# Zhiyu014/GNN-UDS

Hardware: AMD Instinct MI355X
Metric: graph-steps/sec (forward rollout), |V|=10k |E|=12k d=64 (higher is better)
Workload: dtype f32 storage/accumulate, GEMM operands as bf16 hi+lo split (3 MFMA products)

## Files before the change

### gnn_uds_amd/_lib.py

```python
import ctypes
import os

import numpy as np
import torch

_HERE = os.path.dirname(os.path.abspath(__file__))
LIB_PATH = os.environ.get('UDS_LIB_PATH') or os.path.join(_HERE, 'libuds_hip.so')

ABI_VERSION = 22
FLAG_EXACT_FP32, FLAG_REQUIRE_FUSED = 1, 2
PRECISION_FLAGS = {'bf16x3': 0, 'fp32': FLAG_EXACT_FP32}

ACT = {None: 0, 'linear': 0, 'relu': 1, 'tanh': 2, 'sigmoid': 3, 'hard_sigmoid': 4}
_KIND = {'GRU': 0, 'LSTM': 1}

_c_i64 = ctypes.c_int64
_c_int = ctypes.c_int
_c_ptr = ctypes.c_void_p

SYMBOLS = {
    'uds_abi_version': (_c_int, []),
    'uds_last_error': (ctypes.c_char_p, []),
    'uds_csr_create': (_c_int, [_c_ptr, _c_ptr, _c_i64, _c_i64, _c_i64, ctypes.POINTER(_c_ptr)]),
    'uds_csr_destroy': (_c_int, [_c_ptr]),
    'uds_csr_shape': (_c_int, [_c_ptr, ctypes.POINTER(_c_i64), ctypes.POINTER(_c_i64), ctypes.POINTER(_c_i64),
                               ctypes.POINTER(ctypes.c_int32)]),
    'uds_csr_row_order': (_c_int, [_c_ptr, _c_ptr]),
    'uds_dense_act': (_c_int, [_c_ptr, _c_i64, _c_ptr, _c_i64, _c_i64, _c_ptr, _c_ptr, _c_i64, _c_int, _c_ptr, _c_ptr,
                               _c_ptr, _c_ptr, _c_ptr, _c_ptr]),
    'uds_csr_spmm': (_c_int, [_c_ptr, _c_ptr, _c_ptr, _c_i64, _c_i64, _c_ptr, _c_int, _c_ptr, _c_ptr]),
    'uds_conv1d_causal': (_c_int, [_c_ptr, _c_i64, _c_i64, _c_i64, _c_i64, _c_ptr, _c_ptr, _c_i64, _c_i64, _c_i64, _c_int, _c_ptr,
                                   _c_ptr]),
    'uds_dense_cumsum_heads': (_c_int, [_c_ptr, _c_i64, _c_i64, _c_i64, _c_ptr, _c_ptr, _c_ptr, _c_int, _c_ptr, _c_ptr, _c_ptr]),
    'uds_recurrent_fused': (_c_int, [_c_ptr, _c_i64, _c_ptr, _c_ptr, _c_ptr, _c_i64, _c_i64, _c_i64, _c_int, _c_ptr, _c_ptr]),
    'uds_recurrent_fused_supported': (_c_int, [_c_i64, _c_int]),
    'uds_recurrent_forward': (_c_int, [_c_ptr, _c_ptr, _c_ptr, _c_i64, _c_i64, _c_i64, _c_i64, _c_int, _c_ptr, _c_ptr]),
    'uds_attn_sum_pool': (_c_int, [_c_ptr, _c_ptr, _c_i64, _c_i64, _c_i64, _c_ptr, _c_ptr]),
    'uds_attn_sum_pool_pair': (_c_int, [_c_ptr, _c_i64, _c_ptr, _c_i64, _c_ptr, _c_i64, _c_i64, _c_ptr, _c_ptr, _c_ptr]),
    'uds_attn_sum_pool_backward': (_c_int, [_c_ptr, _c_i64, _c_ptr, _c_i64, _c_ptr, _c_ptr, _c_ptr, _c_ptr, _c_i64, _c_i64, _c_ptr, _c_ptr, _c_ptr,
                                            _c_ptr, _c_ptr]),
    'uds_dropout': (_c_int, [_c_ptr, _c_i64, ctypes.c_float, ctypes.c_uint64, ctypes.c_uint64, _c_ptr, _c_ptr]),
    'uds_recurrent_forward_train': (_c_int, [_c_ptr, _c_ptr, _c_ptr, _c_i64, _c_i64, _c_i64, _c_i64, _c_int, _c_ptr, _c_ptr, _c_ptr]),
    'uds_recurrent_backward': (_c_int, [_c_ptr, _c_ptr, _c_ptr, _c_ptr, _c_ptr, _c_ptr, _c_i64, _c_i64, _c_i64, _c_int, _c_ptr, _c_ptr, _c_ptr]),
    'uds_recurrent_bwd_packed_bytes': (_c_i64, [_c_i64, _c_int]),
    'uds_recurrent_pack_bwd': (_c_int, [_c_ptr, _c_i64, _c_int, _c_ptr, _c_ptr]),
    'uds_recurrent_backward_h': (_c_int, [_c_ptr, _c_ptr, _c_ptr, _c_ptr, _c_ptr, _c_ptr, _c_i64, _c_i64, _c_i64, _c_i64, _c_int, _c_ptr, _c_ptr,
                                          _c_ptr]),
    'uds_rowgemm_packed_bytes': (_c_i64, [_c_i64, _c_i64]),
    'uds_rowgemm_pack': (_c_int, [_c_ptr, _c_i64, _c_i64, _c_ptr, _c_ptr]),
    'uds_gat_aggregate_masked': (_c_int, [_c_ptr, _c_ptr, _c_ptr, _c_ptr, _c_ptr, _c_ptr, _c_i64, _c_i64, _c_int, _c_ptr, _c_ptr]),
    'uds_gat_aggregate_coef': (_c_int, [_c_ptr, _c_ptr, _c_ptr, _c_ptr, _c_ptr, _c_ptr, _c_i64, _c_i64, _c_int, _c_ptr, _c_ptr]),
    'uds_diffusion_forward': (_c_int, [_c_ptr, _c_ptr, _c_ptr, _c_ptr, _c_ptr, _c_i64, _c_i64, _c_int, _c_ptr, _c_ptr]),
    'uds_diffusion_backward_workspace_floats': (_c_i64, [_c_i64, _c_i64, _c_i64, _c_i64]),
    'uds_diffusion_backward': (_c_int, [_c_ptr, _c_ptr, _c_ptr, _c_ptr, _c_ptr, _c_ptr, _c_ptr, _c_ptr, _c_ptr, _c_ptr, _c_i64, _c_i64,
                                        _c_i64, _c_int, _c_ptr, _c_ptr, _c_ptr, _c_ptr]),
    'uds_diffusion_forward_m': (_c_int, [_c_ptr, _c_ptr, _c_ptr, _c_ptr, _c_ptr, _c_i64, _c_i64, _c_i64, _c_int, _c_ptr, _c_ptr]),
    'uds_diffusion_backward_m_workspace_floats': (_c_i64, [_c_i64, _c_i64, _c_i64, _c_i64]),
    'uds_diffusion_backward_m': (_c_int, [_c_ptr, _c_ptr, _c_ptr, _c_ptr, _c_ptr, _c_ptr, _c_ptr, _c_ptr, _c_ptr, _c_i64, _c_i64, _c_i64,
                                          _c_int, _c_ptr, _c_ptr, _c_ptr, _c_ptr]),
    'uds_halo_pack': (_c_int, [_c_ptr, _c_i64, _c_ptr, _c_i64, _c_i64, _c_i64, _c_ptr, _c_i64, _c_ptr, _c_i64, _c_ptr, _c_ptr]),
    'uds_halo_unpack': (_c_int, [_c_ptr, _c_i64, _c_i64, _c_ptr, _c_i64, _c_ptr, _c_i64, _c_ptr, _c_i64, _c_ptr, _c_i64, _c_ptr]),
    'uds_halo_pack_all': (_c_int, [_c_ptr, _c_i64, _c_ptr, _c_i64, _c_i64, _c_i64, _c_ptr, _c_i64, _c_ptr, _c_i64, _c_ptr, _c_ptr, _c_i64,
                                   _c_ptr, _c_ptr]),
    'uds_halo_unpack_all': (_c_int, [_c_ptr, _c_i64, _c_i64, _c_ptr, _c_i64, _c_ptr, _c_i64, _c_ptr, _c_ptr, _c_i64, _c_ptr, _c_i64, _c_ptr,
                                     _c_i64, _c_ptr]),
    'uds_halo_pack_clear_all': (_c_int, [_c_ptr, _c_i64, _c_ptr, _c_i64, _c_i64, _c_i64, _c_ptr, _c_i64, _c_ptr, _c_i64, _c_ptr, _c_ptr,
                                         _c_i64, _c_ptr, _c_ptr]),
    'uds_halo_accumulate_all': (_c_int, [_c_ptr, _c_i64, _c_i64, _c_ptr, _c_ptr, _c_i64, _c_ptr, _c_i64, _c_ptr, _c_i64, _c_ptr, _c_ptr,
                                         _c_i64, _c_ptr, _c_i64, _c_ptr, _c_i64, _c_ptr]),
    'uds_remainder_packed_bytes': (_c_i64, [_c_i64, _c_i64]),
    'uds_remainder_pack': (_c_int, [_c_ptr, _c_i64, _c_i64, _c_ptr, _c_ptr]),
    'uds_remainder_workspace_bytes': (_c_i64, [_c_i64, _c_i64, _c_i64, _c_i64]),
    'uds_remainder_forward_dense': (_c_int, [_c_ptr, _c_i64, _c_i64, _c_ptr, _c_i64, _c_ptr, _c_ptr, _c_int, _c_i64, _c_i64, _c_ptr, _c_ptr, _c_ptr]),
    'uds_remainder_forward': (_c_int, [_c_ptr, _c_i64, _c_i64, _c_ptr, _c_i64, _c_i64, _c_ptr, _c_ptr, _c_ptr]),
    'uds_rowgemm_forward': (_c_int, [_c_ptr, _c_i64, _c_i64, _c_i64, _c_i64, _c_ptr, _c_ptr, _c_i64, _c_i64, _c_i64, _c_int, _c_ptr, _c_ptr]),
    'uds_rowgemm_forward_pair': (_c_int, [_c_ptr, _c_i64, _c_ptr, _c_ptr, _c_ptr, _c_ptr, _c_i64, _c_ptr, _c_ptr, _c_ptr, _c_i64, _c_i64, _c_i64, _c_i64,
                                          _c_i64, _c_i64, _c_int, _c_ptr]),
    'uds_rowgemm_forward_cat': (_c_int, [_c_ptr, _c_i64, _c_ptr, _c_i64, _c_i64, _c_i64, _c_i64, _c_ptr, _c_ptr, _c_i64, _c_i64, _c_i64, _c_int,
                                         _c_ptr, _c_i64, _c_i64, _c_ptr]),
    'uds_dense_cumsum': (_c_int, [_c_ptr, _c_i64, _c_i64, _c_i64, _c_ptr, _c_ptr, _c_ptr, _c_int, _c_ptr, _c_ptr]),
    'uds_conv_stack_plan': (_c_int, [_c_i64, _c_i64, _c_i64, _c_int, _c_ptr, _c_ptr, _c_ptr]),
    'uds_conv_stack_forward': (_c_int, [_c_ptr, _c_i64, _c_i64, _c_i64, _c_ptr, _c_i64, _c_ptr, _c_ptr]),
    'uds_cumsum_act': (_c_int, [_c_ptr, _c_ptr, _c_i64, _c_i64, _c_i64, _c_i64, _c_int, _c_ptr, _c_ptr]),
    'uds_flow_balance': (_c_int, [_c_ptr, _c_ptr, _c_ptr, _c_i64, _c_ptr, _c_ptr, _c_ptr, _c_ptr, _c_ptr]),
    'uds_gat_workspace_floats': (_c_i64, [_c_i64, _c_i64, _c_i64]),
    'uds_gat_forward': (_c_int, [_c_ptr, _c_ptr, _c_i64, _c_ptr, _c_i64, _c_i64, _c_ptr, _c_ptr, _c_ptr, _c_ptr, _c_i64,
                                 _c_int, _c_ptr, _c_ptr, _c_ptr]),
    'uds_gat_aggregate': (_c_int, [_c_ptr, _c_ptr, _c_ptr, _c_ptr, _c_ptr, _c_i64, _c_i64, _c_int, _c_ptr, _c_ptr]),
    'uds_gat_backward': (_c_int, [_c_ptr, _c_ptr, _c_ptr, _c_ptr, _c_ptr, _c_ptr, _c_ptr, _c_ptr, _c_ptr, _c_i64, _c_i64, _c_ptr,
                                  _c_ptr, _c_ptr, _c_ptr, _c_ptr, _c_ptr]),
    'uds_gat_backward_coef': (_c_int, [_c_ptr, _c_ptr, _c_ptr, _c_ptr, _c_ptr, _c_ptr, _c_ptr, _c_ptr, _c_ptr, _c_ptr, _c_i64, _c_i64, _c_ptr,
                                       _c_ptr, _c_ptr, _c_ptr, _c_ptr, _c_ptr]),
    'uds_gat_aggregate_ex': (_c_int, [_c_ptr, _c_ptr, _c_ptr, _c_ptr, _c_ptr, _c_ptr, _c_ptr, _c_i64, _c_i64, _c_int, _c_ptr, _c_ptr]),
    'uds_gat_backward_ex': (_c_int, [_c_ptr, _c_ptr, _c_ptr, _c_ptr, _c_ptr, _c_ptr, _c_ptr, _c_ptr, _c_ptr, _c_ptr, _c_ptr, _c_i64, _c_i64,
                                     _c_ptr, _c_ptr, _c_ptr, _c_ptr, _c_ptr, _c_ptr]),
    'uds_gat_aggregate_heads': (_c_int, [_c_ptr, _c_ptr, _c_ptr, _c_ptr, _c_ptr, _c_ptr, _c_ptr, _c_i64, _c_i64, _c_i64, _c_int, _c_int, _c_ptr,
                                         _c_ptr, _c_ptr]),
    'uds_gat_backward_heads': (_c_int, [_c_ptr, _c_ptr, _c_ptr, _c_ptr, _c_ptr, _c_ptr, _c_ptr, _c_ptr, _c_ptr, _c_ptr, _c_ptr, _c_i64, _c_i64,
                                        _c_i64, _c_int, _c_ptr, _c_ptr, _c_ptr, _c_ptr, _c_ptr, _c_ptr]),
    'uds_csr_sddmm': (_c_int, [_c_ptr, _c_ptr, _c_ptr, _c_i64, _c_i64, _c_ptr, _c_ptr]),
    'uds_wgrad_workspace_floats': (_c_i64, [_c_i64, _c_i64, _c_i64, _c_int]),
    'uds_wgrad': (_c_int, [_c_ptr, _c_ptr, _c_i64, _c_i64, _c_i64, _c_i64, _c_i64, _c_i64, _c_int, _c_ptr, _c_ptr, _c_ptr, _c_ptr]),
    'uds_network_create': (_c_int, [_c_ptr, _c_ptr, _c_ptr, _c_ptr, ctypes.POINTER(_c_ptr)]),
    'uds_network_destroy': (_c_int, [_c_ptr]),
    'uds_network_prepare': (_c_int, [_c_ptr, _c_i64, _c_i64]),
    'uds_network_plan_info': (_c_int, [_c_ptr, _c_ptr]),
    'uds_tile_plan_create': (_c_int, [_c_ptr] * 8 + [_c_i64, _c_i64] + [ctypes.c_int32] * 4 + [ctypes.POINTER(_c_ptr)]),
    'uds_tile_plan_destroy': (_c_int, [_c_ptr]),
    'uds_tile_plan_sizes': (_c_int, [_c_ptr, ctypes.POINTER(_c_i64), ctypes.POINTER(_c_i64), _c_ptr]),
    'uds_tile_plan_copy': (_c_int, [_c_ptr, _c_ptr, _c_ptr]),
    'uds_tile_plan_blocks': (_c_int, [_c_ptr, _c_ptr, ctypes.POINTER(_c_i64)]),
    'uds_roll_update': (_c_int, [_c_ptr] * 7 + [_c_i64, _c_ptr, _c_i64, _c_ptr, _c_i64, _c_i64, _c_i64, _c_int, _c_ptr, _c_ptr, _c_ptr, _c_ptr]),
    'uds_predict_tail': (_c_int, [_c_ptr] * 9 + [_c_i64, _c_i64, _c_ptr, _c_ptr, _c_ptr]),
    'uds_predict_tail_workspace_floats': (_c_i64, [_c_i64, _c_i64, _c_i64, _c_i64]),
    'uds_predict_tail_backward': (_c_int, [_c_ptr] * 9 + [_c_i64, _c_i64] + [_c_ptr] * 8),
    'uds_fit_tail': (_c_int, [_c_ptr] * 15 + [_c_i64, _c_i64, _c_i64, _c_int] + [_c_ptr] * 5),
    'uds_fit_tail_workspace_floats': (_c_i64, [_c_i64, _c_i64, _c_i64, _c_i64]),
    'uds_fit_tail_backward': (_c_int, [_c_ptr] * 15 + [_c_i64, _c_i64, _c_i64, _c_int] + [_c_ptr] * 7),
    'uds_spatial_workspace_floats': (_c_i64, [_c_ptr, _c_i64, _c_i64, _c_i64]),
    'uds_spatial_packed_bytes': (_c_i64, []),
    'uds_spatial_pack_weights': (_c_int, [_c_ptr, _c_i64, _c_i64, _c_i64, _c_i64, _c_ptr, _c_ptr]),
    'uds_spatial_layer_forward': (_c_int, [_c_ptr, _c_ptr, _c_ptr, _c_i64, _c_ptr, _c_i64, _c_i64, _c_i64, _c_i64, _c_int,
                                           _c_int, _c_ptr, _c_ptr, _c_ptr, _c_ptr]),
    'uds_spatial_layer_forward_rem': (_c_int, [_c_ptr, _c_ptr, _c_ptr, _c_i64, _c_ptr, _c_i64, _c_ptr, _c_ptr, _c_i64, _c_i64, _c_i64, _c_int, _c_int,
                                      _c_ptr, _c_ptr, _c_ptr, _c_ptr]),
    'uds_spatial_layer_forward_split': (_c_int, [_c_ptr, _c_ptr, _c_ptr, _c_i64, _c_ptr, _c_i64, _c_ptr, _c_i64, _c_ptr, _c_i64, _c_i64,
                                                 _c_i64, _c_i64, _c_int, _c_int, _c_ptr, _c_ptr, _c_ptr, _c_ptr]),
}


class SpatialParams(ctypes.Structure):
    _fields_ = [(n, _c_ptr) for n in ('xe_k', 'xe_b', 'ex_k', 'ex_b', 'ne_n_val', 'ne_e_val',
                                      'gx_k', 'gx_as', 'gx_an', 'gx_b', 'ge_k', 'ge_as', 'ge_an', 'ge_b', 'packed')]


class UdsError(RuntimeError):
    pass


_lib = None


def load():
    global _lib
    if _lib is not None:
        return _lib
    if not os.path.exists(LIB_PATH):
        raise ImportError('%s is missing: the HIP engine is not built (run `python -m gnn_uds_amd.build`); '
                          'gnn_uds_amd has no CPU fallback' % LIB_PATH)
    lib = ctypes.CDLL(LIB_PATH)
    for name, (res, args) in SYMBOLS.items():
        fn = getattr(lib, name)
        fn.restype = res
        fn.argtypes = args
    if lib.uds_abi_version() != ABI_VERSION:
        raise ImportError('libuds_hip.so ABI %d, binding expects %d' % (lib.uds_abi_version(), ABI_VERSION))
    _lib = lib
    return lib


def _check(rc, what):
    if rc != 0:
        msg = load().uds_last_error()
        raise UdsError('%s failed (%d): %s' % (what, rc, msg.decode() if msg else '?'))


def _dev(t, name, allow_none=False):
    if t is None:
        if allow_none:
            return None
        raise UdsError('%s is required' % name)
    if not isinstance(t, torch.Tensor):
        raise UdsError('%s must be a torch.Tensor, got %r' % (name, type(t)))
    if not t.is_cuda:
        raise UdsError('%s is on %s: gnn_uds_amd runs on the MI355X only and has no CPU fallback' % (name, t.device))
    if t.dtype != torch.float32:
        raise UdsError('%s must be float32, got %s' % (name, t.dtype))
    if not t.is_contiguous():
        raise UdsError('%s must be contiguous' % name)
    _same_device(t.device.index, name)
    return t.data_ptr()


def _current_device():
    if not torch.cuda.is_available():
        raise UdsError('no HIP device is visible: gnn_uds_amd runs on the MI355X only and has no CPU fallback')
    return torch.cuda.current_device()


def _same_device(index, what):
    cur = _current_device()
    if index is not None and index != cur:
        raise UdsError('%s lives on cuda:%d but the current device is cuda:%d: call torch.cuda.set_device(%d) (one process per GPU) '
                       'or wrap the call in `with torch.cuda.device(%d):`' % (what, index, cur, index, index))


def _dev_i32(t, name):
    if not isinstance(t, torch.Tensor) or not t.is_cuda or t.dtype != torch.int32 or not t.is_contiguous():
        raise UdsError('%s must be a contiguous int32 HIP tensor' % name)
    _same_device(t.device.index, name)
    return t.data_ptr()


def _stream():
    return torch.cuda.current_stream().cuda_stream


def _nothing_to_launch(t, name, result):
    _dev(t, name)
    return result


def _out(out, shape, like, name):
    if out is None:
        return torch.empty(shape, device=like.device, dtype=torch.float32)
    if tuple(out.shape) != tuple(shape) or out.device != like.device:
        raise UdsError('%s must be %r on %s, got %r on %s' % (name, tuple(shape), like.device, tuple(out.shape), out.device))
    _dev(out, name)
    return out


class CsrHandle:

    def __init__(self, csr):
        lib = load()
        self.n_rows, self.n_cols, self.nnz = int(csr.n_rows), int(csr.n_cols), int(csr.nnz)
        rowptr = np.ascontiguousarray(csr.rowptr, dtype=np.int32)
        col = np.ascontiguousarray(csr.col, dtype=np.int32)
        h = _c_ptr()
        self.device = _current_device()
        _check(lib.uds_csr_create(rowptr.ctypes.data, col.ctypes.data, self.n_rows, self.n_cols, self.nnz,
                                  ctypes.byref(h)), 'uds_csr_create')
        self._h = h
        self._rowptr, self._col = rowptr, col
        self._t = None

    def transposed(self, device):
        if self._t is None:
            rows = np.repeat(np.arange(self.n_rows, dtype=np.int64), np.diff(self._rowptr.astype(np.int64)))
            cols = self._col.astype(np.int64)
            order = np.lexsort((rows, cols))
            t_rowptr = np.zeros(self.n_cols + 1, dtype=np.int64)
            np.add.at(t_rowptr, cols + 1, 1)
            t_rowptr = np.cumsum(t_rowptr)

            class _T:
                pass
            t = _T()
            t.n_rows, t.n_cols, t.nnz = self.n_cols, self.n_rows, self.nnz
            t.rowptr, t.col = t_rowptr.astype(np.int32), rows[order].astype(np.int32)
            self._t = (CsrHandle(t), order.astype(np.int32))
        h, perm = self._t
        if not isinstance(perm, torch.Tensor) or perm.device != torch.device(device):
            perm = torch.as_tensor(np.asarray(perm.cpu() if isinstance(perm, torch.Tensor) else perm), dtype=torch.int32,
                                   device=device)
            self._t = (h, perm)
        return h, perm

    @property
    def ptr(self):
        _same_device(self.device, 'this CSR handle')
        return self._h

    def row_order(self):
        out = np.empty(self.n_rows, dtype=np.int32)
        _check(load().uds_csr_row_order(self._h, out.ctypes.data), 'uds_csr_row_order')
        return out

    def max_degree(self):
        md = ctypes.c_int32()
        _check(load().uds_csr_shape(self._h, None, None, None, ctypes.byref(md)), 'uds_csr_shape')
        return md.value

    def __del__(self):
        h, self._h = getattr(self, '_h', None), None
        if h is not None and _lib is not None:
            _lib.uds_csr_destroy(h)


class NetworkHandle:

    def __init__(self, graph):
        lib = load()
        self.graph = graph
        self.adj = CsrHandle(graph.adj)
        self.edge_adj = CsrHandle(graph.edge_adj)
        self.inc_n = CsrHandle(graph.inc_n)
        self.inc_e = CsrHandle(graph.inc_e)
        h = _c_ptr()
        self.device = _current_device()
        _check(lib.uds_network_create(self.adj.ptr, self.edge_adj.ptr, self.inc_n.ptr, self.inc_e.ptr, ctypes.byref(h)),
               'uds_network_create')
        self._h = h
        self._prepared = {(64, 64)}

    @property
    def ptr(self):
        _same_device(self.device, 'this network handle')
        return self._h

    def prepare(self, fx, fe):
        key = (int(fx), int(fe))
        if key not in self._prepared:
            _check(load().uds_network_prepare(self.ptr, key[0], key[1]), 'uds_network_prepare')
            self._prepared.add(key)

    def plan_info(self):
        info = np.zeros(8, dtype=np.int32)
        _check(load().uds_network_plan_info(self._h, info.ctypes.data), 'uds_network_plan_info')
        keys = ('fused', 'node_tiles', 'link_tiles', 'p_cap', 'q_cap', 'meta_cap', 'lds_bytes', 't_code')
        out = dict(zip(keys, (int(v) for v in info)))
        out['t_node'], out['t_link'] = out['t_code'] // 1000, out['t_code'] % 1000
        return out

    def __del__(self):
        h, self._h = getattr(self, '_h', None), None
        if h is not None and _lib is not None:
            _lib.uds_network_destroy(h)


def tile_plan(graph, t_node=48, t_link=48, p_limit=0, q_limit=0, blocks=False):
    lib = load()
    arrs = []
    for c in (graph.adj, graph.edge_adj, graph.inc_n, graph.inc_e):
        arrs += [np.ascontiguousarray(c.rowptr, dtype=np.int32), np.ascontiguousarray(c.col, dtype=np.int32)]
    h = _c_ptr()
    _check(lib.uds_tile_plan_create(*[a.ctypes.data for a in arrs], graph.n_node, graph.n_edge, t_node, t_link,
                                    p_limit, q_limit, ctypes.byref(h)), 'uds_tile_plan_create')
    try:
        nt, pl = _c_i64(), _c_i64()
        caps = np.zeros(3, dtype=np.int32)
        _check(lib.uds_tile_plan_sizes(h, ctypes.byref(nt), ctypes.byref(pl), caps.ctypes.data), 'uds_tile_plan_sizes')
        hdr = np.zeros((nt.value, 8), dtype=np.int32)
        pool = np.zeros(pl.value, dtype=np.int32)
        _check(lib.uds_tile_plan_copy(h, hdr.ctypes.data, pool.ctypes.data), 'uds_tile_plan_copy')
        blk = None
        if blocks:
            stride = _c_i64()
            if lib.uds_tile_plan_blocks(h, None, ctypes.byref(stride)) == 0:
                blk = np.zeros((nt.value, stride.value), dtype=np.int32)
                _check(lib.uds_tile_plan_blocks(h, blk.ctypes.data, ctypes.byref(stride)), 'uds_tile_plan_blocks')
    finally:
        lib.uds_tile_plan_destroy(h)
    out = dict(p_cap=int(caps[0]), q_cap=int(caps[1]), meta_cap=int(caps[2]))
    if blocks:
        out['blocks'] = blk
    return hdr, pool, out


def dense_act(xa, kernel, bias=None, act='linear', xb=None, attn=None):
    lib = load()
    fa = xa.shape[-1]
    fb = 0 if xb is None else xb.shape[-1]
    rows = xa.numel() // fa
    fo = kernel.shape[-1]
    if kernel.shape[0] != fa + fb:
        raise UdsError('kernel has %d input features, inputs give %d' % (kernel.shape[0], fa + fb))
    if xb is not None and xb.shape[:-1] != xa.shape[:-1]:
        raise UdsError('xa %r and xb %r disagree on leading dims' % (tuple(xa.shape), tuple(xb.shape)))
    out = torch.empty(xa.shape[:-1] + (fo,), device=xa.device, dtype=torch.float32)
    s_self = s_nbr = None
    if attn is not None:
        s_self = torch.empty(xa.shape[:-1], device=xa.device, dtype=torch.float32)
        s_nbr = torch.empty_like(s_self)
    if rows == 0:
        return _nothing_to_launch(xa, 'xa', (out, s_self, s_nbr) if attn is not None else out)
    _check(lib.uds_dense_act(_dev(xa, 'xa'), fa, _dev(xb, 'xb', True), fb, rows, _dev(kernel, 'kernel'),
                             _dev(bias, 'bias', True), fo, ACT[act],
                             _dev(attn[0], 'a_self') if attn else None, _dev(attn[1], 'a_nbr') if attn else None,
                             _dev(out, 'out'), _dev(s_self, 's_self', True), _dev(s_nbr, 's_nbr', True), _stream()),
           'uds_dense_act')
    return (out, s_self, s_nbr) if attn is not None else out


def conv1d_causal(x, kernel, bias=None, dilation=1, act='linear'):
    lib = load()
    if x.dim() != 4 or kernel.dim() != 3 or kernel.shape[1] != x.shape[-1]:
        raise UdsError('conv1d_causal: x %r / kernel %r' % (tuple(x.shape), tuple(kernel.shape)))
    B, T, R, F = x.shape
    taps, _, H = kernel.shape
    out = torch.empty((B, T, R, H), device=x.device, dtype=torch.float32)
    if out.numel() == 0:
        return _nothing_to_launch(x, 'x', out)
    _check(lib.uds_conv1d_causal(_dev(x, 'x'), B, T, R, F, _dev(kernel, 'kernel'), _dev(bias, 'bias', True), taps, dilation, H,
                                 ACT[act], _dev(out, 'out'), _stream()), 'uds_conv1d_causal')
    return out


def recurrent_fused_supported(F, kind):
    return bool(load().uds_recurrent_fused_supported(int(F), _KIND[kind]))


def recurrent_pack(kernel, recurrent_kernel):
    G = recurrent_kernel.shape[1] // 64
    if tuple(recurrent_kernel.shape) != (64, G * 64) or G not in (3, 4) or (kernel is not None and kernel.shape[1] != G * 64):
        raise UdsError('recurrent_pack: kernel %r / recurrent kernel %r (F x G*64 and 64 x G*64 with G = 3 or 4)'
                       % (None if kernel is None else tuple(kernel.shape), tuple(recurrent_kernel.shape)))
    mats = [recurrent_kernel] if kernel is None else [kernel, recurrent_kernel]
    return torch.cat([rowgemm_pack(m[:, 64 * g:64 * (g + 1)].contiguous()) for m in mats for g in range(G)]).contiguous()


def recurrent_fused(x, packed, b_in, b_rec, kind, projected=False):
    lib = load()
    B, T, R, F = x.shape
    out = torch.empty((B, T, R, 64), device=x.device, dtype=torch.float32)
    if out.numel():
        _check(lib.uds_recurrent_fused(_dev(x, 'x'), 0 if projected else F, packed.data_ptr(), _dev(b_in, 'b_in', True), _dev(b_rec, 'b_rec', True),
                                       B, T, R, _KIND[kind], _dev(out, 'out'), _stream()), 'uds_recurrent_fused')
    return out


def attn_sum_pool(x, attn_kernel):
    lib = load()
    B, R, F = x.shape
    k = attn_kernel.reshape(-1).contiguous()
    if k.numel() != F:
        raise UdsError('attn_sum_pool: x %r, attn_kernel %r' % (tuple(x.shape), tuple(attn_kernel.shape)))
    out = torch.empty((B, F), device=x.device, dtype=torch.float32)
    if B:
        _check(lib.uds_attn_sum_pool(_dev(x, 'x'), _dev(k, 'attn_kernel'), B, R, F, _dev(out, 'out'), _stream()), 'uds_attn_sum_pool')
    return out


def _pool_pair_shapes(what, x, e, attn_kernel):
    if x.dim() != 3 or (e is not None and (e.dim() != 3 or e.shape[0] != x.shape[0] or e.shape[2] != x.shape[2])) or attn_kernel.numel() != x.shape[2]:
        raise UdsError('%s: x %r, e %r, attn_kernel %r' % (what, tuple(x.shape), None if e is None else tuple(e.shape), tuple(attn_kernel.shape)))
    if e is not None and e.shape[1] == 0:
        e = None
    return x.shape[0], x.shape[1], 0 if e is None else e.shape[1], x.shape[2], e, attn_kernel.reshape(-1).contiguous()


def attn_sum_pool_pair(x, e, attn_kernel, want_stat=False):
    lib = load()
    B, Rx, Re, F, e, k = _pool_pair_shapes('attn_sum_pool_pair', x, e, attn_kernel)
    out = torch.empty((B, F), device=x.device, dtype=torch.float32)
    stat = torch.empty((B, 2), device=x.device, dtype=torch.float32) if want_stat else None
    if B:
        _check(lib.uds_attn_sum_pool_pair(_dev(x, 'x'), Rx, _dev(e, 'e', True), Re, _dev(k, 'attn_kernel'), B, F, _dev(out, 'out'),
                                          _dev(stat, 'stat', True), _stream()), 'uds_attn_sum_pool_pair')
    return (out, stat) if want_stat else out


def attn_sum_pool_backward(x, e, attn_kernel, out, stat, grad, want_dx=True, want_de=True, want_dk=True, dx=None, de=None, dk=None, dk_ws=None):
    lib = load()
    B, Rx, Re, F, e, k = _pool_pair_shapes('attn_sum_pool_backward', x, e, attn_kernel)
    if tuple(out.shape) != (B, F) or tuple(stat.shape) != (B, 2) or tuple(grad.shape) != (B, F):
        raise UdsError('attn_sum_pool_backward: out %r, stat %r, grad %r for B=%d, F=%d' % (tuple(out.shape), tuple(stat.shape), tuple(grad.shape), B, F))
    dx = _out(dx, (B, Rx, F), x, 'dx') if want_dx else None
    de = _out(de, (B, Re, F), x, 'de') if want_de and e is not None else None
    dk = _out(dk, (F,), x, 'dk') if want_dk else None
    dk_ws = _out(dk_ws, (B, F), x, 'dk_ws') if want_dk else None
    if dx is not None or de is not None or dk is not None:
        _check(lib.uds_attn_sum_pool_backward(_dev(x, 'x'), Rx, _dev(e, 'e', True), Re, _dev(k, 'attn_kernel'), _dev(out, 'out'), _dev(stat, 'stat'),
                                              _dev(grad, 'grad'), B, F, _dev(dx, 'dx', True), _dev(de, 'de', True), _dev(dk_ws, 'dk_ws', True),
                                              _dev(dk, 'dk', True), _stream()), 'uds_attn_sum_pool_backward')
    return dx, de, dk


def dropout(x, rate, seed, offset):
    lib = load()
    x = x.contiguous()
    out = torch.empty_like(x)
    if out.numel():
        _check(lib.uds_dropout(_dev(x, 'x'), x.numel(), float(rate), int(seed) & 0xFFFFFFFFFFFFFFFF, int(offset) & 0xFFFFFFFFFFFFFFFF,
                               _dev(out, 'out'), _stream()), 'uds_dropout')
    return out


def _recurrent_forward(xp, recurrent_kernel, recurrent_bias, kind, train):
    lib = load()
    B, T, R, GH = xp.shape
    G = {'GRU': 3, 'LSTM': 4}[kind]
    H = GH // G
    if GH != G * H or tuple(recurrent_kernel.shape) != (H, GH):
        raise UdsError('recurrent_forward: xp %r, recurrent kernel %r for a %s' % (tuple(xp.shape), tuple(recurrent_kernel.shape), kind))
    out = torch.empty((B, T, R, H), device=xp.device, dtype=torch.float32)
    c = torch.empty_like(out) if train and kind == 'LSTM' else None
    if out.numel():
        entry = 'uds_recurrent_forward_train' if train else 'uds_recurrent_forward'
        _check(getattr(lib, entry)(_dev(xp, 'xp'), _dev(recurrent_kernel, 'recurrent_kernel'), _dev(recurrent_bias, 'recurrent_bias', True),
                                   B, T, R, H, _KIND[kind], _dev(out, 'out'), *([_dev(c, 'c', True)] if train else []), _stream()), entry)
    return out, c


def recurrent_forward_train(xp, recurrent_kernel, recurrent_bias, kind):
    return _recurrent_forward(xp, recurrent_kernel, recurrent_bias, kind, True)


RECURRENT_TRAIN_WIDTHS = tuple(range(16, 129, 16))


def recurrent_bwd_route(units):
    if units == 64:
        return 'uds_recurrent_backward'
    return 'uds_recurrent_backward_h' if units in RECURRENT_TRAIN_WIDTHS else None


# ... 852 lines not shown
```

### gnn_uds_amd/csrc/kernels_fused.hpp

```cpp
#pragma once
#include <hip/hip_runtime.h>
#include <stdint.h>

#include <type_traits>

#include "kernels_dense.hpp"
#include "kernels_sparse.hpp"
#include "tile_plan.hpp"

namespace uds {

typedef __attribute__((ext_vector_type(8))) __bf16 bf16x8;
typedef __attribute__((ext_vector_type(4))) float f32x4;

constexpr int FUSED_H = 32;
constexpr int FUSED_D = 64;
constexpr int FUSED_WAVES = 8;
constexpr int FUSED_U = 4;
constexpr int SEC_STRIDE = FUSED_H + 4;

struct FusedSide {
  const float *prim_in, *sec_in;
  const float *prim_in2, *sec_in2;
  float *out;
  const uint4 *w_small, *w_big;
  const uint4 *w_big32, *w_small32;
  const float *b_small, *a_self, *a_nbr, *b_out, *ne_val;
  int n_prim_glob, n_sec_glob;
  const float *rem;
};

struct FusedArgs {
  FusedSide side[2];
  const int32_t *hdr, *pool;
  const int32_t *blocks;
  int n_tiles, S, chunk, p_cap, q_cap, meta_cap, act, side_mask;
  unsigned long long *dbg;
};

__device__ __forceinline__ int frag_k(int t, int qd, int jj) { return 32 * t + (jj < 4 ? 4 * qd + jj : 16 + 4 * qd + (jj - 4)); }

__global__ void k_pack_weight_frags(const float *__restrict__ W, int K, int F_out, uint4 *__restrict__ out) {
  const int MB = F_out / 16, KT = K / 32;
  const int idx = blockIdx.x * blockDim.x + threadIdx.x;
  if (idx >= KT * MB * 64) return;
  const int lane = idx & 63, m = (idx >> 6) % MB, t = (idx >> 6) / MB;
  const int qd = lane >> 4, f = 16 * m + (lane & 15);
  bf16x8 hi, lo;
#pragma unroll
  for (int jj = 0; jj < 8; ++jj) {
    const float w = W[(int64_t)frag_k(t, qd, jj) * F_out + f];
    const __bf16 h = (__bf16)w;
    hi[jj] = h;
    lo[jj] = (__bf16)(w - (float)h);
  }
  out[((t * MB + m) * 2 + 0) * 64 + lane] = __builtin_bit_cast(uint4, hi);
  out[((t * MB + m) * 2 + 1) * 64 + lane] = __builtin_bit_cast(uint4, lo);
}

__global__ void k_pack_weight_frags32(const float *__restrict__ W, int K, int F_out, uint4 *__restrict__ out) {
  const int MB = F_out / 32, KT = K / 16;
  const int idx = blockIdx.x * blockDim.x + threadIdx.x;
  if (idx >= KT * MB * 64) return;
  const int lane = idx & 63, m = (idx >> 6) % MB, t = (idx >> 6) / MB;
  const int hf = lane >> 5, f = 32 * m + (lane & 31);
  bf16x8 hi, lo;
#pragma unroll
  for (int jj = 0; jj < 8; ++jj) {
    const float w = W[(int64_t)(16 * t + 8 * hf + jj) * F_out + f];
    const __bf16 h = (__bf16)w;
    hi[jj] = h;
    lo[jj] = (__bf16)(w - (float)h);
  }
  out[((t * MB + m) * 2 + 0) * 64 + lane] = __builtin_bit_cast(uint4, hi);
  out[((t * MB + m) * 2 + 1) * 64 + lane] = __builtin_bit_cast(uint4, lo);
}

__device__ __forceinline__ void split8(const float4 &a, const float4 &b, bf16x8 &hi, bf16x8 &lo) {
  typedef float f32x2_t __attribute__((ext_vector_type(2)));
  typedef __bf16 bf16x2_t __attribute__((ext_vector_type(2)));
  const f32x2_t v[4] = {{a.x, a.y}, {a.z, a.w}, {b.x, b.y}, {b.z, b.w}};
  unsigned hw[4], lw[4];
#pragma unroll
  for (int p = 0; p < 4; ++p) {
    const bf16x2_t h = __builtin_convertvector(v[p], bf16x2_t);
    const unsigned hb = __builtin_bit_cast(unsigned, h);
    const f32x2_t hf = {__uint_as_float(hb << 16), __uint_as_float(hb & 0xffff0000u)};
    const bf16x2_t l = __builtin_convertvector(v[p] - hf, bf16x2_t);
    hw[p] = hb;
    lw[p] = __builtin_bit_cast(unsigned, l);
  }
  hi = __builtin_bit_cast(bf16x8, make_uint4(hw[0], hw[1], hw[2], hw[3]));
  lo = __builtin_bit_cast(bf16x8, make_uint4(lw[0], lw[1], lw[2], lw[3]));
}

__device__ __forceinline__ f32x4 mfma3(const bf16x8 &wh, const bf16x8 &wl, const bf16x8 &dh, const bf16x8 &dl, f32x4 acc) {
  acc = __builtin_amdgcn_mfma_f32_16x16x32_bf16(wh, dl, acc, 0, 0, 0);
  acc = __builtin_amdgcn_mfma_f32_16x16x32_bf16(wl, dh, acc, 0, 0, 0);
  acc = __builtin_amdgcn_mfma_f32_16x16x32_bf16(wh, dh, acc, 0, 0, 0);
  return acc;
}

template <int CTRL>
__device__ __forceinline__ float row_dpp(float v) {
  const int x = __builtin_bit_cast(int, v);
  return __builtin_bit_cast(float, __builtin_amdgcn_update_dpp(x, x, CTRL, 0xf, 0xf, true));
}
__device__ __forceinline__ float row16_max(float v) {
  v = fmaxf(v, row_dpp<0xB1>(v));
  v = fmaxf(v, row_dpp<0x4E>(v));
  v = fmaxf(v, row_dpp<0x124>(v));
  v = fmaxf(v, row_dpp<0x128>(v));
  return v;
}
__device__ __forceinline__ float row16_sum(float v) {
  v += row_dpp<0xB1>(v);
  v += row_dpp<0x4E>(v);
  v += row_dpp<0x124>(v);
  v += row_dpp<0x128>(v);
  return v;
}

#define UDS_DPP4(op, ctrl)                                                      \
  op " %0, %0, %0 " ctrl " row_mask:0xf bank_mask:0xf bound_ctrl:1\n\t"       \
  op " %1, %1, %1 " ctrl " row_mask:0xf bank_mask:0xf bound_ctrl:1\n\t"       \
  op " %2, %2, %2 " ctrl " row_mask:0xf bank_mask:0xf bound_ctrl:1\n\t"       \
  op " %3, %3, %3 " ctrl " row_mask:0xf bank_mask:0xf bound_ctrl:1\n\t"
#define UDS_DPP4_FIRST(op, ctrl)                                                \
  op " %0, %4, %4 " ctrl " row_mask:0xf bank_mask:0xf bound_ctrl:1\n\t"       \
  op " %1, %5, %5 " ctrl " row_mask:0xf bank_mask:0xf bound_ctrl:1\n\t"       \
  op " %2, %6, %6 " ctrl " row_mask:0xf bank_mask:0xf bound_ctrl:1\n\t"       \
  op " %3, %7, %7 " ctrl " row_mask:0xf bank_mask:0xf bound_ctrl:1\n\t"
__device__ __forceinline__ void row16_max4(const float (&in)[4], float (&out)[4]) {
  asm("s_nop 1\n\t" UDS_DPP4_FIRST("v_max_f32_dpp", "quad_perm:[1,0,3,2]") UDS_DPP4("v_max_f32_dpp", "quad_perm:[2,3,0,1]")
      UDS_DPP4("v_max_f32_dpp", "row_ror:4") UDS_DPP4("v_max_f32_dpp", "row_ror:8")
      : "=&v"(out[0]), "=&v"(out[1]), "=&v"(out[2]), "=&v"(out[3])
      : "v"(in[0]), "v"(in[1]), "v"(in[2]), "v"(in[3]));
}
__device__ __forceinline__ void row16_sum4(const float (&in)[4], float (&out)[4]) {
  asm("s_nop 1\n\t" UDS_DPP4_FIRST("v_add_f32_dpp", "quad_perm:[1,0,3,2]") UDS_DPP4("v_add_f32_dpp", "quad_perm:[2,3,0,1]")
      UDS_DPP4("v_add_f32_dpp", "row_ror:4") UDS_DPP4("v_add_f32_dpp", "row_ror:8")
      : "=&v"(out[0]), "=&v"(out[1]), "=&v"(out[2]), "=&v"(out[3])
      : "v"(in[0]), "v"(in[1]), "v"(in[2]), "v"(in[3]));
}

__device__ __forceinline__ float quarters_sum(float v) {
  const unsigned u = __float_as_uint(v);
  const auto a = __builtin_amdgcn_permlane16_swap(u, u, false, false);
  const float s = __uint_as_float(a[0]) + __uint_as_float(a[1]);
  const unsigned w = __float_as_uint(s);
  const auto b = __builtin_amdgcn_permlane32_swap(w, w, false, false);
  return __uint_as_float(b[0]) + __uint_as_float(b[1]);
}

template <int ACT>
__device__ __forceinline__ float fused_act(float v, int act_rt) {
  if constexpr (ACT == UDS_ACT_RELU) return __int_as_float(max(__float_as_int(v), 0));
  else if constexpr (ACT == UDS_ACT_LINEAR) return v;
  else return apply_act(v, act_rt);
}

__device__ __forceinline__ void lds_barrier() { asm volatile("s_waitcnt lgkmcnt(0)\n\ts_barrier" ::: "memory"); }

template <int N, int I = 0, class F>
__device__ __forceinline__ void static_for(F &&f) {
  if constexpr (I < N) {
    f(std::integral_constant<int, I>{});
    static_for<N, I + 1>(f);
  }
}

constexpr int P3_SLOTS = 2;

template <int K>
__device__ __forceinline__ int row16_bcast(int v) {
  static_assert(K >= 0 && K < 16, "lane inside a 16-lane row");
  return __builtin_amdgcn_update_dpp(v, v, 0x150 + K, 0xf, 0xf, true);
}

__device__ __forceinline__ void wait_all_but(int n) {
  switch (n) {
    case 0: asm volatile("s_waitcnt vmcnt(0)" ::: "memory"); break;
    case 1: asm volatile("s_waitcnt vmcnt(1)" ::: "memory"); break;
    case 2: asm volatile("s_waitcnt vmcnt(2)" ::: "memory"); break;
    case 3: asm volatile("s_waitcnt vmcnt(3)" ::: "memory"); break;
    default: asm volatile("s_waitcnt vmcnt(4)" ::: "memory"); break;
  }
}
// ... 534 lines not shown
```

### gnn_uds_amd/csrc/kernels_fused_ws.hpp

```cpp
#pragma once
#include "kernels_fused.hpp"

namespace uds {

constexpr int WS_NY = 4, WS_NX = FUSED_WAVES - WS_NY;
constexpr int WS_XPRIO = 1;
constexpr int WS_OCT_WD = 4;
constexpr int WS_OCT_GRP = 1;

inline int64_t fused_ws_lds_bytes(int p_cap, int q_cap, int meta_cap) {
  return 4 * ((int64_t)meta_cap + 4 * p_cap + 3 * FUSED_D + FUSED_H + 2 * (int64_t)q_cap * SEC_STRIDE + 2 * (int64_t)p_cap * FUSED_D);
}

template <int IMM>
__device__ __forceinline__ void ws_gld16(f32x4 &dst, const float *base, unsigned voff) {
  asm volatile("global_load_dwordx4 %0, %1, %2 offset:%3" : "=v"(dst) : "v"(voff), "s"(base), "n"(IMM) : "memory");
}
__device__ __forceinline__ void ws_pin4(f32x4 &a0, f32x4 &a1, f32x4 &a2, f32x4 &a3) {
  asm volatile("" : "+v"(a0), "+v"(a1), "+v"(a2), "+v"(a3));
}
__device__ __forceinline__ void row8_max4(const float (&in)[4], float (&out)[4]) {
  asm("s_nop 1\n\t" UDS_DPP4_FIRST("v_max_f32_dpp", "quad_perm:[1,0,3,2]") UDS_DPP4("v_max_f32_dpp", "quad_perm:[2,3,0,1]")
      UDS_DPP4("v_max_f32_dpp", "row_half_mirror")
      : "=&v"(out[0]), "=&v"(out[1]), "=&v"(out[2]), "=&v"(out[3])
      : "v"(in[0]), "v"(in[1]), "v"(in[2]), "v"(in[3]));
}
__device__ __forceinline__ void row8_sum4(const float (&in)[4], float (&out)[4]) {
  asm("s_nop 1\n\t" UDS_DPP4_FIRST("v_add_f32_dpp", "quad_perm:[1,0,3,2]") UDS_DPP4("v_add_f32_dpp", "quad_perm:[2,3,0,1]")
      UDS_DPP4("v_add_f32_dpp", "row_half_mirror")
      : "=&v"(out[0]), "=&v"(out[1]), "=&v"(out[2]), "=&v"(out[3])
      : "v"(in[0]), "v"(in[1]), "v"(in[2]), "v"(in[3]));
}
template <int HI>
__device__ __forceinline__ unsigned ws_add_half(unsigned pk, unsigned base) {
  unsigned r;
  if (HI) asm("v_add_u32_sdwa %0, %1, %2 dst_sel:DWORD dst_unused:UNUSED_PAD src0_sel:WORD_1 src1_sel:DWORD" : "=v"(r) : "v"(pk), "v"(base));
  else asm("v_add_u32_sdwa %0, %1, %2 dst_sel:DWORD dst_unused:UNUSED_PAD src0_sel:WORD_0 src1_sel:DWORD" : "=v"(r) : "v"(pk), "v"(base));
  return r;
}
__device__ __forceinline__ void ws_vmcnt(int n) {
  switch (n) {
    case 0: asm volatile("s_waitcnt vmcnt(0)" ::: "memory"); break;
    case 1: asm volatile("s_waitcnt vmcnt(1)" ::: "memory"); break;
    case 2: asm volatile("s_waitcnt vmcnt(2)" ::: "memory"); break;
    case 3: asm volatile("s_waitcnt vmcnt(3)" ::: "memory"); break;
    case 4: asm volatile("s_waitcnt vmcnt(4)" ::: "memory"); break;
    case 5: asm volatile("s_waitcnt vmcnt(5)" ::: "memory"); break;
    case 6: asm volatile("s_waitcnt vmcnt(6)" ::: "memory"); break;
    case 7: asm volatile("s_waitcnt vmcnt(7)" ::: "memory"); break;
    default: asm volatile("s_waitcnt vmcnt(8)" ::: "memory"); break;
  }
}

template <int ACT>
__global__ __launch_bounds__(FUSED_WAVES * 64, 2) void k_fused_ws(FusedArgs a) {
  constexpr int NT = FUSED_WAVES * 64, NY = WS_NY, NX = WS_NX;
  constexpr int FP = 64, FS = 64;
  constexpr int U = FUSED_U;
  extern __shared__ __attribute__((aligned(16))) int32_t smem[];

  const int tid = threadIdx.x, lane = tid & 63;
  const int wave = __builtin_amdgcn_readfirstlane(tid >> 6);
  const bool team_y = wave < NY;
  const int yw = wave, xw = wave - NY;

  const int W = gridDim.x, b = blockIdx.x;
  const int q8 = W / 8, r8 = W % 8, xcd = b % 8;
  const int w = (xcd < r8 ? xcd * (q8 + 1) : r8 * (q8 + 1) + (xcd - r8) * q8) + b / 8;
  const int tile = w % a.n_tiles;
  const int chunk_id = w / a.n_tiles;
  const int s_begin = chunk_id * a.chunk;
  const int s_end = min(a.S, (chunk_id + 1) * a.chunk);
  const int sd = __builtin_amdgcn_readfirstlane(a.hdr[tile * TILE_HDR_INTS + 6]);
  if (!((a.side_mask >> sd) & 1)) return;
  const FusedSide &S_ = a.side[sd];

  float *s_self = reinterpret_cast<float *>(smem + a.meta_cap);
  float *s_nbr = s_self + 2 * a.p_cap;
  float *attn = s_nbr + 2 * a.p_cap;
  float *sec = attn + 3 * FUSED_D + FUSED_H;
  float *hx = sec + 2 * a.q_cap * SEC_STRIDE;
  const int sec_buf = a.q_cap * SEC_STRIDE, hx_buf = a.p_cap * FUSED_D;

  {
    const uint4 *src = reinterpret_cast<const uint4 *>(a.blocks + (int64_t)tile * a.meta_cap);
    uint4 *dst = reinterpret_cast<uint4 *>(smem);
    for (int i = tid; i < a.meta_cap / 4; i += NT) dst[i] = src[i];
  }
  if (tid < FUSED_D) {
    attn[tid] = S_.a_self[tid] * 1.44269504088896340736f;
    attn[FUSED_D + tid] = S_.a_nbr[tid] * 1.44269504088896340736f;
    if (tid < FUSED_H) attn[2 * FUSED_D + tid] = S_.b_small ? S_.b_small[tid] : 0.f;
    attn[2 * FUSED_D + FUSED_H + tid] = S_.b_out ? S_.b_out[tid] : 0.f;
  }
  __syncthreads();
  const int n_own = __builtin_amdgcn_readfirstlane(smem[0]), n_prim = __builtin_amdgcn_readfirstlane(smem[1]),
            n_sec = __builtin_amdgcn_readfirstlane(smem[2]), flags = __builtin_amdgcn_readfirstlane(smem[3]),
            n_ovf = __builtin_amdgcn_readfirstlane(smem[4]), n_adj = __builtin_amdgcn_readfirstlane(smem[5]),
            inc_width = __builtin_amdgcn_readfirstlane(smem[7]);
  const EllOffsets off = ell_offsets(n_own, n_prim, n_sec, flags, n_ovf, n_adj);
  const int32_t *prim_ids = smem + off.prim;
  const int32_t *sec_ids = smem + off.sec;
  const uint32_t *inc_loc = reinterpret_cast<const uint32_t *>(smem + off.inc_loc);
  int32_t *inc_w = smem + off.inc_w;
  const f32x4 *inc_val4 = reinterpret_cast<const f32x4 *>(inc_w);
  const unsigned char *adj_b = reinterpret_cast<const unsigned char *>(smem + off.adj);
  const int32_t *ovf_ptr = smem + off.ovf_ptr, *ovf_loc = smem + off.ovf_loc;
  int32_t *ovf_w = smem + off.ovf_w;
  const int32_t *adj_ptr = smem + off.adj_ptr, *adj_loc = smem + off.adj_loc;

  for (int i = tid; i < ELL_INC * n_prim; i += NT) {
    const int k = inc_w[i];
    reinterpret_cast<float *>(inc_w)[i] = k >= 0 ? S_.ne_val[k] : 0.f;
  }
  if (flags & ELL_FLAG_INC_OVF)
    for (int i = tid; i < n_ovf; i += NT) reinterpret_cast<float *>(ovf_w)[i] = S_.ne_val[ovf_w[i]];
  const float *ovf_val = reinterpret_cast<const float *>(ovf_w);

#ifdef UDS_PHASE_TIMING
  unsigned long long tm_[8] = {0, 0, 0, 0, 0, 0, 0, 0}, tl_ = clock64();
  const unsigned long long rt0_ = __builtin_amdgcn_s_memrealtime(), mt0_ = tl_;
#define WS_STAMP(k) do { const unsigned long long n_ = clock64(); tm_[k] += n_ - tl_; tl_ = n_; } while (0)
#define WS_DUMP() do { if (a.dbg && lane == 0) { unsigned long long *o = a.dbg + ((size_t)blockIdx.x * 8 + wave) * 16; \
    for (int q_ = 0; q_ < 7; ++q_) o[q_] = tm_[q_]; o[12] = wave; \
    o[15] = ((__builtin_amdgcn_s_memrealtime() - rt0_) << 32) | ((clock64() - mt0_) & 0xffffffffull); \
    o[7] = 1ull | ((unsigned long long)sd << 8) | ((unsigned long long)n_own << 16) | ((unsigned long long)n_prim << 32) | ((unsigned long long)n_sec << 48); } } while (0)
#else
#define WS_STAMP(k) do { } while (0)
#define WS_DUMP() do { } while (0)
#endif
  const int64_t sec_stride = (int64_t)S_.n_sec_glob * FS, prim_stride = (int64_t)S_.n_prim_glob * FP;
  const int n_snap = s_end - s_begin;

  __syncthreads();
  if (team_y) {
    typedef float f32x16 __attribute__((ext_vector_type(16)));
    constexpr int KT32 = (FP + FUSED_H) / 16, KX32 = FP / 16, MB32 = FUSED_D / 32;
    static_assert(NY == 4, "one 32-row block per Y wave: four waves cover p_cap = 128");
    const int n32 = lane & 31, hf = lane >> 5;
    bf16x8 wh[KT32][MB32], wl[KT32][MB32];
#pragma unroll
    for (int t = 0; t < KT32; ++t)
#pragma unroll
      for (int m = 0; m < MB32; ++m) {
        wh[t][m] = __builtin_bit_cast(bf16x8, S_.w_big32[((t * MB32 + m) * 2 + 0) * 64 + lane]);
        wl[t][m] = __builtin_bit_cast(bf16x8, S_.w_big32[((t * MB32 + m) * 2 + 1) * 64 + lane]);
      }
    const int lrow = 32 * yw + n32;
    const bool valid = lrow < n_prim;
    const int lr = min(lrow, n_prim - 1);
    const unsigned prow = (unsigned)prim_ids[lr] * FP + 8u * hf;
    f32x4 pp[2 * KX32];
    const bool has_rem = S_.rem != nullptr;
    const unsigned rrow = (unsigned)prim_ids[lr] * FUSED_H + 8u * hf;
    f32x4 rm[4] = {f32x4{0.f, 0.f, 0.f, 0.f}, f32x4{0.f, 0.f, 0.f, 0.f}, f32x4{0.f, 0.f, 0.f, 0.f}, f32x4{0.f, 0.f, 0.f, 0.f}};
    const int64_t rem_stride = (int64_t)S_.n_prim_glob * FUSED_H;
    const unsigned ag_locs = inc_loc[lr];
    const f32x4 ag_vals = inc_val4[lr];
    __builtin_amdgcn_s_waitcnt(0x0F70);
    if (n_snap > 0) {
      const float *base = S_.prim_in + s_begin * prim_stride;
      static_for<2 * KX32>([&](auto i_) {
        constexpr int i = decltype(i_)::value;
        pp[i] = *reinterpret_cast<const f32x4 *>(base + prow + 16 * (i >> 1) + 4 * (i & 1));
      });
      if (has_rem) {
        const float *rb = S_.rem + s_begin * rem_stride + rrow;
        rm[0] = *reinterpret_cast<const f32x4 *>(rb);
        rm[1] = *reinterpret_cast<const f32x4 *>(rb + 4);
        rm[2] = *reinterpret_cast<const f32x4 *>(rb + 16);
        rm[3] = *reinterpret_cast<const f32x4 *>(rb + 20);
      }
    }
    WS_STAMP(0);
    lds_barrier();

    auto mfma3_32 = [&](const bf16x8 &a_h, const bf16x8 &a_l, const bf16x8 &d_h, const bf16x8 &d_l, f32x16 acc) __attribute__((always_inline)) {
      acc = __builtin_amdgcn_mfma_f32_32x32x16_bf16(a_h, d_l, acc, 0, 0, 0);
      acc = __builtin_amdgcn_mfma_f32_32x32x16_bf16(a_l, d_h, acc, 0, 0, 0);
      acc = __builtin_amdgcn_mfma_f32_32x32x16_bf16(a_h, d_h, acc, 0, 0, 0);
      return acc;
    };
    for (int k = 0; k <= n_snap; ++k) {
      if (k < n_snap && 32 * yw < n_prim) {
        const bool more = k + 1 < n_snap;
        const float *next = S_.prim_in + (s_begin + k + 1) * prim_stride;
        const float *secr = sec + (k & 1) * sec_buf;
        float *hxw = hx + (k & 1) * hx_buf;
        float *ssw = s_self + (k & 1) * a.p_cap, *snw = s_nbr + (k & 1) * a.p_cap;
        bf16x8 dh[KT32], dl[KT32];
        static_for<KX32>([&](auto t_) {
          constexpr int t = decltype(t_)::value;
          const f32x4 u0 = pp[2 * t], u1 = pp[2 * t + 1];
          split8(make_float4(u0[0], u0[1], u0[2], u0[3]), make_float4(u1[0], u1[1], u1[2], u1[3]), dh[t], dl[t]);
        });
        if (more)
          static_for<2 * KX32>([&](auto i_) {
            constexpr int i = decltype(i_)::value;
            pp[i] = *reinterpret_cast<const f32x4 *>(next + prow + 16 * (i >> 1) + 4 * (i & 1));
          });
        f32x16 acc[MB32];
#pragma unroll
        for (int m = 0; m < MB32; ++m)
#pragma unroll
          for (int r = 0; r < 16; ++r) acc[m][r] = 0.f;
#pragma unroll
        for (int t = 0; t < KX32; ++t)
#pragma unroll
          for (int m = 0; m < MB32; ++m) acc[m] = mfma3_32(wh[t][m], wl[t][m], dh[t], dl[t], acc[m]);
        float4 g0 = make_float4(rm[0][0], rm[0][1], rm[0][2], rm[0][3]), g1 = make_float4(rm[1][0], rm[1][1], rm[1][2], rm[1][3]),
               g2 = make_float4(rm[2][0], rm[2][1], rm[2][2], rm[2][3]), g3 = make_float4(rm[3][0], rm[3][1], rm[3][2], rm[3][3]);
        if (more && has_rem) {
          const float *rb = S_.rem + (s_begin + k + 1) * rem_stride + rrow;
          rm[0] = *reinterpret_cast<const f32x4 *>(rb);
          rm[1] = *reinterpret_cast<const f32x4 *>(rb + 4);
          rm[2] = *reinterpret_cast<const f32x4 *>(rb + 16);
          rm[3] = *reinterpret_cast<const f32x4 *>(rb + 20);
        }
        auto fma4 = [&](float4 &g, float wv, const float4 &u) { g.x = fmaf(wv, u.x, g.x); g.y = fmaf(wv, u.y, g.y); g.z = fmaf(wv, u.z, g.z); g.w = fmaf(wv, u.w, g.w); };
        auto add_row = [&](unsigned la, float wa) {
          const float *ra = secr + la * SEC_STRIDE + 8 * hf;
          const float4 u0 = *reinterpret_cast<const float4 *>(ra), u1 = *reinterpret_cast<const float4 *>(ra + 4);
          const float4 u2 = *reinterpret_cast<const float4 *>(ra + 16), u3 = *reinterpret_cast<const float4 *>(ra + 20);
          fma4(g0, wa, u0); fma4(g1, wa, u1); fma4(g2, wa, u2); fma4(g3, wa, u3);
        };
        add_row(ag_locs & 0xffu, ag_vals[0]);
        add_row((ag_locs >> 8) & 0xffu, ag_vals[1]);
        if (inc_width > 2) {
          add_row((ag_locs >> 16) & 0xffu, ag_vals[2]);
          add_row(ag_locs >> 24, ag_vals[3]);
        }
        if (flags & ELL_FLAG_INC_OVF)
          for (int p = ovf_ptr[lr]; p < ovf_ptr[lr + 1]; ++p) add_row((unsigned)ovf_loc[p], ovf_val[p]);
        split8(g0, g1, dh[KX32], dl[KX32]);
        split8(g2, g3, dh[KX32 + 1], dl[KX32 + 1]);
#pragma unroll
        for (int t = KX32; t < KT32; ++t)
#pragma unroll
          for (int m = 0; m < MB32; ++m) acc[m] = mfma3_32(wh[t][m], wl[t][m], dh[t], dl[t], acc[m]);
        float ps = 0.f, pn = 0.f;
#pragma unroll
        for (int m = 0; m < MB32; ++m)
#pragma unroll
          for (int gq = 0; gq < 4; ++gq) {
            const f32x4 as4 = *reinterpret_cast<const f32x4 *>(attn + 32 * m + 8 * gq + 4 * hf);
            const f32x4 an4 = *reinterpret_cast<const f32x4 *>(attn + FUSED_D + 32 * m + 8 * gq + 4 * hf);
#pragma unroll
            for (int q = 0; q < 4; ++q) {
              ps = fmaf(acc[m][4 * gq + q], as4[q], ps);
              pn = fmaf(acc[m][4 * gq + q], an4[q], pn);
            }
          }
        ps += __shfl_xor(ps, 32);
        pn += __shfl_xor(pn, 32);
        if (valid) {
          if (hf == 0) {
            ssw[lrow] = ps;
            snw[lrow] = pn;
          }
#pragma unroll
          for (int m = 0; m < MB32; ++m)
#pragma unroll
            for (int gq = 0; gq < 4; ++gq) {
              const f32x4 o = {acc[m][4 * gq], acc[m][4 * gq + 1], acc[m][4 * gq + 2], acc[m][4 * gq + 3]};
              *reinterpret_cast<f32x4 *>(hxw + lrow * FUSED_D + (((8 * m + 2 * gq + hf) ^ (lrow & 7)) << 2)) = o;
            }
        }
      }
      WS_STAMP(1);
      lds_barrier();
      WS_STAMP(2);
    }
    WS_DUMP();
  } else {
    __builtin_amdgcn_s_setprio(WS_XPRIO);
    typedef float f32x16 __attribute__((ext_vector_type(16)));
    constexpr int KS32 = FS / 16, SJ32 = (8 + NX - 1) / NX;
    const int n32 = lane & 31, hf = lane >> 5;
    bf16x8 w1h[KS32], w1l[KS32];
#pragma unroll
    for (int t = 0; t < KS32; ++t) {
      w1h[t] = __builtin_bit_cast(bf16x8, S_.w_small32[(t * 2 + 0) * 64 + lane]);
      w1l[t] = __builtin_bit_cast(bf16x8, S_.w_small32[(t * 2 + 1) * 64 + lane]);
    }
    unsigned srow[SJ32];
#pragma unroll
    for (int j = 0; j < SJ32; ++j) srow[j] = ((unsigned)sec_ids[min((xw + NX * j) * 32 + n32, n_sec - 1)] * FS + 8u * hf) * 4u;
    f32x4 sp[SJ32][2 * KS32];
    auto load_sec_at = [&](const float *base) __attribute__((always_inline)) {
      static_for<SJ32>([&](auto j_) {
        constexpr int j = decltype(j_)::value;
        ws_gld16<0>(sp[j][0], base, srow[j]);
        ws_gld16<16>(sp[j][1], base, srow[j]);
        ws_gld16<64>(sp[j][2], base, srow[j]);
        ws_gld16<80>(sp[j][3], base, srow[j]);
        ws_gld16<128>(sp[j][4], base, srow[j]);
        ws_gld16<144>(sp[j][5], base, srow[j]);
        ws_gld16<192>(sp[j][6], base, srow[j]);
        ws_gld16<208>(sp[j][7], base, srow[j]);
      });
    };
    auto load_sec = [&](int s) __attribute__((always_inline)) { load_sec_at(S_.sec_in + s * sec_stride); };
    const int ro = lane >> 3, c8 = lane & 7, hf8 = ro & 1;
    int p3_dmax[U];
    unsigned p3_pk[U][4];
    unsigned p3_jb4 = 0;
    int n_st = 0;
#pragma unroll
    for (int u = 0; u < U; ++u) {
      const int i = 8 * (NX * u + xw) + ro;
      const int ic = min(i, n_own - 1);
      int dmx;
      if (flags & ELL_FLAG_LONG_ROWS) {
        dmx = i < n_own ? adj_ptr[ic + 1] - adj_ptr[ic] : 0;
      } else {
        const unsigned long long m0 = __ballot(i < n_own && adj_b[ic * ELL_ADJ + c8] != 0xFF);
        const unsigned long long m1 = __ballot(i < n_own && adj_b[ic * ELL_ADJ + 8 + c8] != 0xFF);
        dmx = __builtin_popcountll((m0 >> (8 * ro)) & 0xffull) + __builtin_popcountll((m1 >> (8 * ro)) & 0xffull);
      }
#pragma unroll
      for (int o = 8; o < 64; o <<= 1) dmx = max(dmx, __shfl_xor(dmx, o));
      p3_dmax[u] = __builtin_amdgcn_readfirstlane(dmx);
#pragma unroll
      for (int k2 = 0; k2 < 4; ++k2) {
        unsigned pk = 0;
#pragma unroll
        for (int h = 0; h < 2; ++h) {
          const unsigned jb = adj_b[ic * ELL_ADJ + 2 * k2 + h];
          const unsigned j = (i < n_own && jb != 0xFFu) ? jb : 0u;
          pk |= (j * (FUSED_D * 4) + (((j & 7) ^ c8) << 4)) << (16 * h);
        }
        p3_pk[u][k2] = pk;
      }
      p3_jb4 |= (i < n_own ? (unsigned)adj_b[i * ELL_ADJ + c8] : 0xFFu) << (8 * u);
      if (8 * (NX * u + xw) < n_own) n_st += 2;
    }
    const float *bias_l = attn + 2 * FUSED_D + FUSED_H + 4 * c8;
    __builtin_amdgcn_s_waitcnt(0x0F70);

    auto phase1 = [&](int buf) __attribute__((always_inline)) {
      float *secw = sec + buf * sec_buf;
      static_for<SJ32>([&](auto j_) {
        constexpr int j = decltype(j_)::value;
        const int blk = xw + NX * j;
        if (blk * 32 < n_sec) {
          f32x16 acc;
#pragma unroll
          for (int gq = 0; gq < 4; ++gq) {
            const f32x4 b4 = *reinterpret_cast<const f32x4 *>(attn + 2 * FUSED_D + 8 * gq + 4 * hf);
#pragma unroll
            for (int q = 0; q < 4; ++q) acc[4 * gq + q] = b4[q];
          }
          static_for<KS32>([&](auto t_) {
            constexpr int t = decltype(t_)::value;
            const f32x4 u0 = sp[j][2 * t], u1 = sp[j][2 * t + 1];
            bf16x8 dh, dl;
            split8(make_float4(u0[0], u0[1], u0[2], u0[3]), make_float4(u1[0], u1[1], u1[2], u1[3]), dh, dl);
            acc = __builtin_amdgcn_mfma_f32_32x32x16_bf16(w1h[t], dl, acc, 0, 0, 0);
            acc = __builtin_amdgcn_mfma_f32_32x32x16_bf16(w1l[t], dh, acc, 0, 0, 0);
            acc = __builtin_amdgcn_mfma_f32_32x32x16_bf16(w1h[t], dh, acc, 0, 0, 0);
          });
          const int lrow = blk * 32 + n32;
          if (lrow < n_sec) {
#pragma unroll
            for (int gq = 0; gq < 4; ++gq) {
              f32x4 o;
#pragma unroll
              for (int q = 0; q < 4; ++q) o[q] = fused_act<ACT>(acc[4 * gq + q], a.act);
              *reinterpret_cast<f32x4 *>(secw + lrow * SEC_STRIDE + 8 * gq + 4 * hf) = o;
            }
          }
        }
      });
    };
    auto pin_rows = [&]() __attribute__((always_inline)) {
      static_for<SJ32>([&](auto j_) {
        constexpr int j = decltype(j_)::value;
        ws_pin4(sp[j][0], sp[j][1], sp[j][2], sp[j][3]);
        ws_pin4(sp[j][4], sp[j][5], sp[j][6], sp[j][7]);
      });
    };

    if (n_snap > 0) {
      load_sec(s_begin);
      ws_vmcnt(0);
      pin_rows();
      phase1(0);
      if (n_snap > 1) load_sec(s_begin + 1);
    }
    WS_STAMP(0);
    lds_barrier();

    auto phase3o = [&](float *out_snap, int buf) __attribute__((always_inline)) {
      const float *hxr = hx + buf * hx_buf;
      const float *ssr = s_self + buf * a.p_cap, *snr = s_nbr + buf * a.p_cap;
      int d0 = p3_dmax[0], d1 = p3_dmax[1], d2 = p3_dmax[2], d3 = p3_dmax[3];
      asm volatile("" : "+s"(d0), "+s"(d1), "+s"(d2), "+s"(d3));
      const int e3 = d3, e2 = max(e3, d2), e1 = max(e2, d1), e0 = max(e1, d0);
      if (e0 == 0) return;

      float ss[U], lg0[U], lg1[U], w0[U], w1[U], den[U];
      bool ok[U], has0[U], has1[U];
      unsigned jb0[U], jb1[U];
      int joff1[U];
#pragma unroll
      for (int u = 0; u < U; ++u) {
        ok[u] = 8 * (NX * u + xw) + ro < n_own;
        jb0[u] = (p3_jb4 >> (8 * u)) & 0xFFu;
        ss[u] = ssr[8 * (NX * u + xw) + ro];
      }
#pragma unroll
      for (int u = 0; u < U; ++u) has0[u] = ok[u] && jb0[u] != 0xFFu;
      f32x4 acc0[U], acc1[U];
#pragma unroll
      for (int u = 0; u < U; ++u) acc0[u] = acc1[u] = f32x4{0.f, 0.f, 0.f, 0.f};
      if (e0 <= 16) {
        const bool ext = e0 > 8;
        float sn[U];
#pragma unroll
        for (int u = 0; u < U; ++u) sn[u] = snr[jb0[u]];
        asm volatile("" : "+v"(sn[0]), "+v"(sn[1]), "+v"(sn[2]), "+v"(sn[3]));
#pragma unroll
        for (int u = 0; u < U; ++u) {
          const float sv = ss[u] + sn[u];
          lg0[u] = has0[u] ? fmaxf(sv, 0.2f * sv) : -INFINITY;
        }
        float mx[U];
        row8_max4(lg0, mx);
        if (ext) {
          float m1[U];
#pragma unroll
          for (int u = 0; u < U; ++u) jb1[u] = adj_b[(8 * (NX * u + xw) + ro) * ELL_ADJ + 8 + c8];
          asm volatile("" : "+v"(jb1[0]), "+v"(jb1[1]), "+v"(jb1[2]), "+v"(jb1[3]));
#pragma unroll
          for (int u = 0; u < U; ++u) sn[u] = snr[jb1[u]];
          asm volatile("" : "+v"(sn[0]), "+v"(sn[1]), "+v"(sn[2]), "+v"(sn[3]));
#pragma unroll
          for (int u = 0; u < U; ++u) {
            has1[u] = ok[u] && jb1[u] != 0xFFu;
            const int j1 = has1[u] ? (int)jb1[u] : 0;
            joff1[u] = j1 * (FUSED_D * 4) + ((j1 & 7) << 4);
            const float sv = ss[u] + sn[u];
            lg1[u] = has1[u] ? fmaxf(sv, 0.2f * sv) : -INFINITY;
          }
          row8_max4(lg1, m1);
#pragma unroll
          for (int u = 0; u < U; ++u) mx[u] = fmaxf(mx[u], m1[u]);
        }
#pragma unroll
        for (int u = 0; u < U; ++u) w0[u] = has0[u] ? __builtin_amdgcn_exp2f(lg0[u] - mx[u]) : 0.f;
        row8_sum4(w0, den);
        if (ext) {
          float d1s[U];
#pragma unroll
          for (int u = 0; u < U; ++u) w1[u] = has1[u] ? __builtin_amdgcn_exp2f(lg1[u] - mx[u]) : 0.f;
          row8_sum4(w1, d1s);
#pragma unroll
          for (int u = 0; u < U; ++u) den[u] += d1s[u];
        }
        typedef const __attribute__((address_space(3))) f32x4 *lds_f4;
        const unsigned hxa0 = lds_addr(hxr) + 128 * hf8, hxa1 = lds_addr(hxr) + 128 - 128 * hf8;
        const int cx = c8 << 4;
        const int bp = (lane & 56) << 2;
        using I1 = std::integral_constant<int, 1>; using I2 = std::integral_constant<int, 2>;
        using I3 = std::integral_constant<int, 3>; using I4 = std::integral_constant<int, 4>;
        auto step = [&](auto SET_, auto K_, auto A_) __attribute__((always_inline)) {
          constexpr int SET = decltype(SET_)::value, K = decltype(K_)::value, A = decltype(A_)::value,
                        Wd = (8 - K < WS_OCT_WD ? 8 - K : WS_OCT_WD);
          constexpr int G = WS_OCT_GRP;
          static_for<(A + G - 1) / G>([&](auto g_) {
            constexpr int u0 = decltype(g_)::value * G, GA = (A - u0 < G ? A - u0 : G);
            f32x4 h0[GA][Wd], h1[GA][Wd];
            static_for<GA>([&](auto u_) {
              constexpr int ul = decltype(u_)::value, u = u0 + ul;
              static_for<Wd>([&](auto i_) {
                constexpr int i = decltype(i_)::value, k = K + i;
                unsigned ad = 0;
                if (SET) ad = (unsigned)__builtin_amdgcn_ds_bpermute(bp + 4 * k, joff1[u]) ^ cx;
                unsigned ad0, ad1;
                if (SET) {
                  ad0 = ad + hxa0;
                  ad1 = ad + hxa1;
                } else {
                  ad0 = ws_add_half<k & 1>(p3_pk[u][k >> 1], hxa0);
                  ad1 = ws_add_half<k & 1>(p3_pk[u][k >> 1], hxa1);
                }
                h0[ul][i] = *(lds_f4)(uintptr_t)ad0;
                h1[ul][i] = *(lds_f4)(uintptr_t)ad1;
              });
            });
            static_for<GA>([&](auto u_) {
              constexpr int ul = decltype(u_)::value, u = u0 + ul;
              static_for<Wd>([&](auto i_) {
                constexpr int i = decltype(i_)::value, k = K + i;
                float wv;
                if (SET) wv = __int_as_float(__builtin_amdgcn_ds_bpermute(bp + 4 * k, __float_as_int(w1[u])));
                else {
                  const int wi = __float_as_int(w0[u]);
                  int t = __builtin_amdgcn_update_dpp(wi, wi, 0x150 + k, 0xf, 0xf, true);
                  t = __builtin_amdgcn_update_dpp(t, wi, 0x150 + 8 + k, 0xf, 0xc, false);
                  wv = __int_as_float(t);
                }
#pragma unroll
                for (int q = 0; q < 4; ++q) {
                  acc0[u][q] = fmaf(wv, h0[ul][i][q], acc0[u][q]);
                  acc1[u][q] = fmaf(wv, h1[ul][i][q], acc1[u][q]);
                }
              });
            });
          });
        };
        static_for<(8 + WS_OCT_WD - 1) / WS_OCT_WD>([&](auto t_) {
          constexpr int K = decltype(t_)::value * WS_OCT_WD;
          using IK = std::integral_constant<int, K>;
          using S0 = std::integral_constant<int, 0>;
          if (K < e3) step(S0{}, IK{}, I4{});
          else if (K < e2) step(S0{}, IK{}, I3{});
          else if (K < e1) step(S0{}, IK{}, I2{});
          else if (K < e0) step(S0{}, IK{}, I1{});
        });
        if (ext)
          static_for<(8 + WS_OCT_WD - 1) / WS_OCT_WD>([&](auto t_) {
            constexpr int K = decltype(t_)::value * WS_OCT_WD;
            using IK = std::integral_constant<int, K>;
            using S1 = std::integral_constant<int, 1>;
            if (K + 8 < e3) step(S1{}, IK{}, I4{});
            else if (K + 8 < e2) step(S1{}, IK{}, I3{});
            else if (K + 8 < e1) step(S1{}, IK{}, I2{});
            else if (K + 8 < e0) step(S1{}, IK{}, I1{});
          });
      } else {
#pragma unroll
        for (int u = 0; u < U; ++u) {
          const int i = 8 * (NX * u + xw) + ro;
          const int b0 = i < n_own ? adj_ptr[i] : 0;
          const int dg = i < n_own ? adj_ptr[i + 1] - b0 : 0;
          float mx = -INFINITY;
          for (int p = b0; p < b0 + dg; ++p) mx = fmaxf(mx, leaky02(ss[u] + snr[adj_loc[p]]));
          den[u] = 0.f;
          for (int p = b0; p < b0 + dg; ++p) {
            const int jj = adj_loc[p];
            const float wv = __builtin_amdgcn_exp2f(leaky02(ss[u] + snr[jj]) - mx);
            const f32x4 v0 = *reinterpret_cast<const f32x4 *>(hxr + jj * FUSED_D + 32 * hf8 + ((c8 ^ (jj & 7)) << 2));
            const f32x4 v1 = *reinterpret_cast<const f32x4 *>(hxr + jj * FUSED_D + 32 - 32 * hf8 + ((c8 ^ (jj & 7)) << 2));
            den[u] += wv;
#pragma unroll
            for (int q = 0; q < 4; ++q) {
              acc0[u][q] = fmaf(wv, v0[q], acc0[u][q]);
              acc1[u][q] = fmaf(wv, v1[q], acc1[u][q]);
            }
          }
        }
      }
      f32x4 bo0 = *reinterpret_cast<const f32x4 *>(bias_l + 32 * hf8), bo1 = *reinterpret_cast<const f32x4 *>(bias_l + 32 - 32 * hf8);
      int pid[U];
#pragma unroll
      for (int u = 0; u < U; ++u) pid[u] = prim_ids[8 * (NX * u + xw) + ro];
      asm volatile("" : "+v"(pid[0]), "+v"(pid[1]), "+v"(pid[2]), "+v"(pid[3]), "+v"(bo0), "+v"(bo1));
      float *out_s = out_snap + (4 * c8 + 32 * hf8);
      const int o1_off = 32 - 64 * hf8;
#pragma unroll
      for (int u = 0; u < U; ++u) {
        if (ok[u]) {
          const float inv = __builtin_amdgcn_rcpf(den[u]);
          f32x4 o0, o1;
#pragma unroll
          for (int q = 0; q < 4; ++q) {
            o0[q] = fused_act<ACT>(fmaf(acc0[u][q], inv, bo0[q]), a.act);
            o1[q] = fused_act<ACT>(fmaf(acc1[u][q], inv, bo1[q]), a.act);
          }
          float *orow = out_s + (int64_t)pid[u] * FUSED_D;
          *reinterpret_cast<f32x4 *>(orow) = o0;
          *reinterpret_cast<f32x4 *>(orow + o1_off) = o1;
        }
      }
    };
    const float *sec_next = S_.sec_in + (int64_t)(s_begin + 2) * sec_stride;
    float *out_next = S_.out + (int64_t)s_begin * S_.n_prim_glob * FUSED_D;
    const int64_t out_stride = (int64_t)S_.n_prim_glob * FUSED_D;
    for (int k = 0; k <= n_snap; ++k) {
      if (k + 1 < n_snap) {
        ws_vmcnt(k >= 2 ? n_st : 0);
        pin_rows();
        phase1((k + 1) & 1);
        if (k + 2 < n_snap) load_sec_at(sec_next);
        sec_next += sec_stride;
      }
      WS_STAMP(3);
      if (k >= 1) {
        phase3o(out_next, (k - 1) & 1);
        out_next += out_stride;
        WS_STAMP(4);
      }
      WS_STAMP(1);
      lds_barrier();
      WS_STAMP(2);
    }
    WS_DUMP();
  }
}

}
```

### gnn_uds_amd/csrc/tile_plan.hpp

```cpp
#pragma once
#include <algorithm>
#include <cmath>
#include <cstdint>
#include <numeric>
#include <vector>

namespace uds {

struct HostCsr {
  int64_t n_rows = 0, n_cols = 0;
  std::vector<int32_t> rowptr, col;
};

constexpr int TILE_HDR_INTS = 8;
inline int tile_block_ints(int meta_cap) { return (TILE_HDR_INTS + meta_cap + 3) & ~3; }

struct SidePlan {
  int n_tiles = 0;
  int p_cap = 0, q_cap = 0, meta_cap = 0;
  std::vector<int32_t> hdr;
  std::vector<int32_t> pool;
  std::vector<int32_t> key;
  std::vector<int32_t> bfs_index;
};
// ... 255 lines not shown
    plan.pool.insert(plan.pool.end(), adj_loc.begin(), adj_loc.end());
    const int32_t meta_len = (int32_t)plan.pool.size() - off;
    while (plan.pool.size() % 4) plan.pool.push_back(0);

    std::vector<int32_t> ks;
    for (int32_t r : own) {
      if (node_bfs) {
        for (int32_t p = inc.rowptr[r]; p < inc.rowptr[r + 1]; ++p) ks.push_back((*node_bfs)[inc.col[p]]);
      } else {
        ks.push_back(plan.bfs_index[r]);
      }
    }
    int32_t key = INT32_MAX;
    if (!ks.empty()) {
      std::nth_element(ks.begin(), ks.begin() + ks.size() / 2, ks.end());
      key = ks[ks.size() / 2];
    }
    plan.key.push_back(key);
    const int32_t h[TILE_HDR_INTS] = {(int32_t)own.size(), (int32_t)prim.size(), (int32_t)sec.size(), (int32_t)inc_loc.size(),
                                      (int32_t)adj_loc.size(), off, side, meta_len};
    plan.hdr.insert(plan.hdr.end(), h, h + TILE_HDR_INTS);
    plan.p_cap = std::max(plan.p_cap, ((int)prim.size() + 15) / 16 * 16);
    plan.q_cap = std::max(plan.q_cap, ((int)sec.size() + 15) / 16 * 16);
    plan.meta_cap = std::max(plan.meta_cap, (meta_len + 3) / 4 * 4);
    for (int32_t r : prim) ploc[r] = -1;
    for (int32_t q : sec) sloc[q] = -1;
  }
  return plan;
}

#ifdef __HIPCC__
#define UDS_HD __host__ __device__
#else
#define UDS_HD
#endif
constexpr int ELL_INC = 4, ELL_ADJ = 16;
constexpr int ELL_FLAG_INC_OVF = 1, ELL_FLAG_LONG_ROWS = 2;
UDS_HD inline int a4(int x) { return (x + 3) & ~3; }

struct EllOffsets {
  int prim, sec, inc_loc, inc_w, adj, ovf_ptr, ovf_loc, ovf_w, adj_ptr, adj_loc, len;
};
UDS_HD inline EllOffsets ell_offsets(int n_own, int n_prim, int n_sec, int flags, int n_ovf, int n_adj) {
  EllOffsets o{};
  int p = TILE_HDR_INTS;
  o.prim = p; p = a4(p + n_prim);
  o.sec = p; p = a4(p + n_sec);
  o.inc_loc = p; p = a4(p + n_prim);
  o.inc_w = p; p += ELL_INC * n_prim;
  o.adj = p; p += (ELL_ADJ / 4) * n_own;
  if (flags & ELL_FLAG_INC_OVF) {
    o.ovf_ptr = p; p = a4(p + n_prim + 1);
    o.ovf_loc = p; p = a4(p + n_ovf);
    o.ovf_w = p; p = a4(p + n_ovf);
  }
  if (flags & ELL_FLAG_LONG_ROWS) {
    o.adj_ptr = p; p = a4(p + n_own + 1);
    o.adj_loc = p; p = a4(p + n_adj);
  }
  o.len = p;
  return o;
}

struct TileView {
  int n_own, n_prim, n_sec, n_inc, n_adj, side;
  const int32_t *prim, *sec, *inc_ptr, *inc_loc, *inc_w, *adj_ptr, *adj_loc;
};
inline TileView tile_view(const int32_t *hd, const int32_t *pool) {
  TileView v{hd[0], hd[1], hd[2], hd[3], hd[4], hd[6], nullptr, nullptr, nullptr, nullptr, nullptr, nullptr, nullptr};
  v.prim = pool + hd[5];
  v.sec = v.prim + v.n_prim;
  v.inc_ptr = v.sec + v.n_sec;
  v.inc_loc = v.inc_ptr + v.n_prim + 1;
  v.inc_w = v.inc_loc + v.n_inc;
  v.adj_ptr = v.inc_w + v.n_inc;
  v.adj_loc = v.adj_ptr + v.n_own + 1;
  return v;
}
inline void ell_shape(const TileView &v, int &flags, int &n_ovf, int &inc_width) {
  flags = 0; n_ovf = 0; inc_width = 0;
  for (int i = 0; i < v.n_prim; ++i) {
    const int d = v.inc_ptr[i + 1] - v.inc_ptr[i];
    inc_width = std::max(inc_width, std::min(d, ELL_INC));
    if (d > ELL_INC) { flags |= ELL_FLAG_INC_OVF; n_ovf += d - ELL_INC; }
  }
  for (int i = 0; i < v.n_own; ++i)
    if (v.adj_ptr[i + 1] - v.adj_ptr[i] > ELL_ADJ) flags |= ELL_FLAG_LONG_ROWS;
}
inline bool ell_fits(const int32_t *hd) { return hd[1] <= 255 && hd[2] <= 256; }
inline int ell_block_len(const int32_t *hd, const int32_t *pool) {
  const TileView v = tile_view(hd, pool);
  int flags, n_ovf, w;
  ell_shape(v, flags, n_ovf, w);
  return ell_offsets(v.n_own, v.n_prim, v.n_sec, flags, n_ovf, v.n_adj).len;
}
inline int ell_block_cap(const std::vector<int32_t> &hdr, const std::vector<int32_t> &pool, int n_tiles) {
  int cap = 4;
  for (int t = 0; t < n_tiles; ++t) {
    const int32_t *hd = hdr.data() + (size_t)t * TILE_HDR_INTS;
    if (!ell_fits(hd)) return -1;
    cap = std::max(cap, ell_block_len(hd, pool.data()));
  }
  return cap;
}
inline void build_ell_blocks(const std::vector<int32_t> &hdr, const std::vector<int32_t> &pool, int n_tiles, int stride,
                             std::vector<int32_t> &out) {
  out.assign(std::max<size_t>((size_t)stride * n_tiles, 4), 0);
  for (int t = 0; t < n_tiles; ++t) {
    const int32_t *hd = hdr.data() + (size_t)t * TILE_HDR_INTS;
    const TileView v = tile_view(hd, pool.data());
    int flags, n_ovf, w;
    ell_shape(v, flags, n_ovf, w);
    const EllOffsets o = ell_offsets(v.n_own, v.n_prim, v.n_sec, flags, n_ovf, v.n_adj);
    int32_t *b = out.data() + (size_t)stride * t;
    const int32_t h[TILE_HDR_INTS] = {v.n_own, v.n_prim, v.n_sec, flags, n_ovf, (flags & ELL_FLAG_LONG_ROWS) ? v.n_adj : 0, v.side, w};
    std::copy(h, h + TILE_HDR_INTS, b);
    std::copy(v.prim, v.prim + v.n_prim, b + o.prim);
    std::copy(v.sec, v.sec + v.n_sec, b + o.sec);
    int q = 0;
    if (flags & ELL_FLAG_INC_OVF) b[o.ovf_ptr] = 0;
    for (int i = 0; i < v.n_prim; ++i) {
      uint32_t locs = 0;
      for (int k = 0; k < ELL_INC; ++k) {
        const int p = v.inc_ptr[i] + k;
        const bool has = p < v.inc_ptr[i + 1];
        if (has) locs |= (uint32_t)v.inc_loc[p] << (8 * k);
        b[o.inc_w + ELL_INC * i + k] = has ? v.inc_w[p] : -1;
      }
      b[o.inc_loc + i] = (int32_t)locs;
      if (flags & ELL_FLAG_INC_OVF) {
        for (int p = v.inc_ptr[i] + ELL_INC; p < v.inc_ptr[i + 1]; ++p, ++q) {
          b[o.ovf_loc + q] = v.inc_loc[p];
          b[o.ovf_w + q] = v.inc_w[p];
        }
        b[o.ovf_ptr + i + 1] = q;
      }
    }
    for (int i = 0; i < v.n_own; ++i)
      for (int c = 0; c < ELL_ADJ / 4; ++c) {
        uint32_t word = 0;
        for (int k = 0; k < 4; ++k) {
          const int p = v.adj_ptr[i] + 4 * c + k;
          word |= (uint32_t)(p < v.adj_ptr[i + 1] ? v.adj_loc[p] : 0xFF) << (8 * k);
        }
        b[o.adj + (ELL_ADJ / 4) * i + c] = (int32_t)word;
      }
    if (flags & ELL_FLAG_LONG_ROWS) {
      std::copy(v.adj_ptr, v.adj_ptr + v.n_own + 1, b + o.adj_ptr);
      std::copy(v.adj_loc, v.adj_loc + v.n_adj, b + o.adj_loc);
    }
  }
}

inline int64_t fused_lds_bytes(int p_cap, int q_cap, int meta_cap, int h, int d, int fp, int fs) {
  const int64_t weights = 16 * 64 * 2 * ((int64_t)(fs / 32) * (h / 16) + (int64_t)((fp + h) / 32) * (d / 16));
  const int64_t stage = std::max<int64_t>(4 * ((int64_t)q_cap * fs + (int64_t)p_cap * fp), weights);
  const int64_t cold = (fp > 64 ? (d / 16) * 2 * 1024 : 0) + (fs > 64 ? (h / 16) * 2 * 1024 : 0);
  return 4 * ((int64_t)meta_cap + 2 * p_cap + 2 * d + h + (int64_t)q_cap * (h + 4) + (int64_t)p_cap * d) + cold + stage;
}

struct NetworkPlan {
  SidePlan side[2];
  std::vector<int32_t> hdr;
  std::vector<int32_t> pool;
  int n_tiles = 0, p_cap = 0, q_cap = 0, meta_cap = 0, t_max[2] = {0, 0};
};

inline NetworkPlan build_network_plan(const HostCsr &adj, const HostCsr &eadj, const HostCsr &inc_n, const HostCsr &inc_e,
                                      int t_node, int t_link, int p_limit = 0, int q_limit = 0) {
  NetworkPlan np;
  np.t_max[0] = t_node;
  np.t_max[1] = t_link;
  np.side[0] = build_side_plan(adj, inc_n, t_node, 0, nullptr, p_limit, q_limit);
  np.side[1] = build_side_plan(eadj, inc_e, t_link, 1, &np.side[0].bfs_index, p_limit, q_limit);
  struct Ref { int32_t key, side, idx; };
  std::vector<Ref> refs;
  for (int s = 0; s < 2; ++s)
    for (int t = 0; t < np.side[s].n_tiles; ++t) refs.push_back({np.side[s].key[t], s, t});
  std::stable_sort(refs.begin(), refs.end(), [](const Ref &a, const Ref &b) { return a.key < b.key; });
  const int32_t base1 = (int32_t)np.side[0].pool.size();
  np.pool = np.side[0].pool;
  np.pool.insert(np.pool.end(), np.side[1].pool.begin(), np.side[1].pool.end());
  for (const Ref &r : refs) {
    const int32_t *h = &np.side[r.side].hdr[(size_t)r.idx * TILE_HDR_INTS];
    for (int i = 0; i < TILE_HDR_INTS; ++i) np.hdr.push_back(i == 5 ? h[i] + (r.side ? base1 : 0) : h[i]);
  }
  np.n_tiles = (int)refs.size();
  np.p_cap = std::max(np.side[0].p_cap, np.side[1].p_cap);
  np.q_cap = std::max(np.side[0].q_cap, np.side[1].q_cap);
  np.meta_cap = std::max(np.side[0].meta_cap, np.side[1].meta_cap);
  return np;
}

}
```

### gnn_uds_amd/csrc/uds_hip.hip

```cpp
#include <hip/hip_runtime.h>

#include <algorithm>
#include <cmath>
#include <cstdarg>
#include <cstdio>
#include <cstring>
#include <initializer_list>
#include <new>
#include <numeric>
#include <string>
#include <vector>

#include "../../include/uds_hip.h"
#include <cstdlib>

#include "kernels_dense.hpp"
#include "kernels_sparse.hpp"
#include "kernels_pool.hpp"
#include "kernels_backward.hpp"
#include "kernels_fused.hpp"
#include "kernels_fused_ws.hpp"
#include "kernels_rowgemm.hpp"
#include "kernels_wgrad.hpp"
#include "kernels_conv_stream.hpp"
#include "kernels_conv_stack.hpp"
#include "kernels_fused128.hpp"
#include "kernels_gemm.hpp"
#include "kernels_recurrent.hpp"
#include "kernels_recurrent_bwd.hpp"
#include "kernels_tail.hpp"
#include "kernels_fit_tail.hpp"
#include "tile_plan.hpp"

namespace {

thread_local std::string g_err;

int fail(int code, const char *fmt, ...) {
  char buf[512];
  va_list ap;
  va_start(ap, fmt);
  vsnprintf(buf, sizeof buf, fmt, ap);
  va_end(ap);
  g_err = buf;
  return code;
}

int launched(const char *entry, hipError_t e) {
  if (e != hipSuccess) return fail(UDS_EHIP, "%s: launch -> %s", entry, hipGetErrorString(e));
  return UDS_OK;
}

#define UDS_HIP_TRY(call)                                                             \
  do {                                                                                 \
    hipError_t e_ = (call);                                                            \
    if (e_ != hipSuccess) return fail(UDS_EHIP, "%s -> %s", #call, hipGetErrorString(e_)); \
  } while (0)

#define UDS_REQUIRE(cond, ...) \
  do {                         \
    if (!(cond)) return fail(UDS_EINVAL, __VA_ARGS__); \
  } while (0)

inline bool aligned16(const void *p) { return (reinterpret_cast<uintptr_t>(p) & 15u) == 0; }
inline int64_t align4(int64_t floats) { return (floats + 3) & ~int64_t(3); }

}

struct uds_csr {
  int64_t n_rows = 0, n_cols = 0, nnz = 0;
  int32_t max_degree = 0;
  int32_t *d_rowptr = nullptr, *d_col = nullptr, *d_order = nullptr, *d_rowidx = nullptr;
  std::vector<int32_t> h_order;
  uds::HostCsr host;
};

struct uds_tile_plan {
  uds::NetworkPlan plan;
};

struct uds_plan_slot {
  bool built = false;
  bool ok = false;
  int fp = 0, fs = 0;
  uds::NetworkPlan plan;
  int32_t *d_hdr = nullptr, *d_pool = nullptr;
  int32_t *d_hdr_side[2] = {nullptr, nullptr};
  int32_t *d_blocks = nullptr, *d_blocks_side[2] = {nullptr, nullptr};
  int blk_cap = 0;
  int64_t lds_bytes = 0;
};

struct uds_network {
  const uds_csr *adj = nullptr, *edge_adj = nullptr, *inc_n = nullptr, *inc_e = nullptr;
  uds_plan_slot slot[7];
};

namespace {

constexpr int64_t FUSED_LDS_BUDGET = 160 * 1024;
constexpr int WS_BIG32_OFF = 2 * (768 + 2048), WS_BIG32_LEN = 6 * 2 * 2 * 64;
constexpr int WS_SMALL32_OFF = WS_BIG32_OFF + 2 * WS_BIG32_LEN, WS_SMALL32_LEN = 4 * 1 * 2 * 64;
constexpr int64_t PACKED_WEIGHT_FLOATS = 2 * (2048 + 6144) * 4;

inline int slot_index(int fp, int fs) {
  if (fp == 128 || fs == 128) return fp == 128 ? (fs == 128 ? 4 : 5) : 6;
  return (fp > 64 ? 2 : 0) + (fs > 64 ? 1 : 0);
}

bool plan_network(const uds::HostCsr &adj, const uds::HostCsr &eadj, const uds::HostCsr &inc_n, const uds::HostCsr &inc_e,
                  int fp, int fs, uds::NetworkPlan &out, int64_t &lds, int &blk_cap) {
  const int cand[][2] = {{128, 208}, {128, 192}, {128, 176}, {128, 160}, {128, 144}, {112, 160}, {112, 144}, {96, 144}, {96, 128},
                         {80, 128}, {64, 96}, {48, 64}, {32, 48}, {16, 32}};
  for (const auto &c : cand) {
    int p_lim = c[0], q_lim = c[1];
#ifdef UDS_KNOBS
    if (const char *ov = std::getenv("UDS_PLIM")) p_lim = std::min(p_lim, std::atoi(ov));
    if (const char *ov = std::getenv("UDS_QLIM")) q_lim = std::min(q_lim, std::atoi(ov));
#endif
    if (uds::fused_lds_bytes(p_lim, q_lim, 0, uds::FUSED_H, uds::FUSED_D, fp, fs) > FUSED_LDS_BUDGET) continue;
    const int t = std::min(p_lim, 4 * uds::FUSED_WAVES * uds::FUSED_U);
    out = uds::build_network_plan(adj, eadj, inc_n, inc_e, t, t, p_lim, q_lim);
    blk_cap = uds::ell_block_cap(out.hdr, out.pool, out.n_tiles);
    if (blk_cap < 0) continue;
    lds = uds::fused_lds_bytes(out.p_cap, out.q_cap, blk_cap, uds::FUSED_H, uds::FUSED_D, fp, fs);
    if (lds <= FUSED_LDS_BUDGET && out.p_cap <= 4 * uds::FUSED_WAVES * uds::FUSED_U) return true;
  }
  return false;
}

bool plan_network128(const uds::HostCsr &adj, const uds::HostCsr &eadj, const uds::HostCsr &inc_n, const uds::HostCsr &inc_e, int fp, int fs,
                     uds::NetworkPlan &out, int64_t &lds) {
  const int cand[][2] = {{64, 128}, {64, 112}, {64, 96}, {64, 80}, {64, 64}, {48, 64}, {32, 48}, {16, 32}};
  for (const auto &c : cand) {
    const int p_lim = c[0], q_lim = c[1];
    if (uds::fused128_lds_bytes(p_lim, q_lim, 0, fp, fs) > FUSED_LDS_BUDGET) continue;
    const int t = std::min(p_lim, 4 * uds::FUSED_WAVES * uds::F128_U);
    out = uds::build_network_plan(adj, eadj, inc_n, inc_e, t, t, p_lim, q_lim);
    lds = uds::fused128_lds_bytes(out.p_cap, out.q_cap, out.meta_cap, fp, fs);
    if (lds <= FUSED_LDS_BUDGET && out.p_cap <= 4 * uds::FUSED_WAVES * uds::F128_U) return true;
  }
  return false;
}

}

namespace {

template <int FP, int FS, int ACT>
hipError_t launch_fused128_act(const uds::FusedArgs &a, int grid, int64_t lds, hipStream_t st) {
  static unsigned long long attr_done = 0;
  if (hipError_t e = uds::set_max_lds_once(reinterpret_cast<const void *>(&uds::k_fused_cs<128, FP, FS, uds::FUSED_WAVES, ACT>), (int)FUSED_LDS_BUDGET, attr_done); e != hipSuccess) return e;
  hipLaunchKernelGGL((uds::k_fused_cs<128, FP, FS, uds::FUSED_WAVES, ACT>), dim3(grid), dim3(uds::FUSED_WAVES * 64), (size_t)lds, st, a);
  return hipGetLastError();
}

template <int FP, int FS>
hipError_t launch_fused128(const uds::FusedArgs &a, int grid, int64_t lds, hipStream_t st) {
  if (a.act == UDS_ACT_RELU) return launch_fused128_act<FP, FS, UDS_ACT_RELU>(a, grid, lds, st);
  return launch_fused128_act<FP, FS, -1>(a, grid, lds, st);
}

template <int FP, int FS, int ACT>
hipError_t launch_fused_act(const uds::FusedArgs &a, int grid, int64_t lds, hipStream_t st) {
  static unsigned long long attr_done = 0;
  if (hipError_t e = uds::set_max_lds_once(reinterpret_cast<const void *>(&uds::k_fused_tile<FP, FS, ACT>), (int)FUSED_LDS_BUDGET, attr_done); e != hipSuccess) return e;
  hipLaunchKernelGGL((uds::k_fused_tile<FP, FS, ACT>), dim3(grid), dim3(uds::FUSED_WAVES * 64), (size_t)lds, st, a);
  return hipGetLastError();
}

template <int ACT>
hipError_t launch_fused_ws_act(const uds::FusedArgs &a, int grid, int64_t lds, hipStream_t st) {
  static unsigned long long attr_done = 0;
  if (hipError_t e = uds::set_max_lds_once(reinterpret_cast<const void *>(&uds::k_fused_ws<ACT>), (int)FUSED_LDS_BUDGET, attr_done); e != hipSuccess) return e;
  hipLaunchKernelGGL((uds::k_fused_ws<ACT>), dim3(grid), dim3(uds::FUSED_WAVES * 64), (size_t)lds, st, a);
  return hipGetLastError();
}
hipError_t launch_fused_ws(const uds::FusedArgs &a, int grid, int64_t lds, hipStream_t st) {
  if (a.act == UDS_ACT_RELU) return launch_fused_ws_act<UDS_ACT_RELU>(a, grid, lds, st);
  return launch_fused_ws_act<-1>(a, grid, lds, st);
}

template <int FP, int FS>
hipError_t launch_fused(const uds::FusedArgs &a, int grid, int64_t lds, hipStream_t st) {
  if (a.act == UDS_ACT_RELU) return launch_fused_act<FP, FS, UDS_ACT_RELU>(a, grid, lds, st);
  return launch_fused_act<FP, FS, -1>(a, grid, lds, st);
}

int64_t pick_chunk(int64_t S, int64_t working_tiles) {
  int64_t chunk = S, best = INT64_MAX;
  for (int64_t c = 1; c <= S; ++c) {
    const int64_t rounds = (((S + c - 1) / c) * working_tiles + 255) / 256;
    const int64_t cost = rounds * (3 + 2 * c);
    if (cost < best || (cost == best && c < chunk)) {
      best = cost;
      chunk = c;
    }
  }
  return chunk;
}

hipError_t pack_weights(const float *W, int K, int F_out, uint4 *out, hipStream_t st) {
  const int total = (K / 32) * (F_out / 16) * 64;
  hipLaunchKernelGGL(uds::k_pack_weight_frags, dim3((total + 255) / 256), dim3(256), 0, st, W, K, F_out, out);
  return hipGetLastError();
}

}

extern "C" {

int uds_abi_version(void) { return UDS_ABI_VERSION; }
const char *uds_last_error(void) { return g_err.c_str(); }

int uds_csr_create(const int32_t *rowptr, const int32_t *col, int64_t n_rows, int64_t n_cols,
                   int64_t nnz, uds_csr_t **out) {
  UDS_REQUIRE(out != nullptr, "uds_csr_create: out is NULL");
  *out = nullptr;
  UDS_REQUIRE(rowptr != nullptr && (col != nullptr || nnz == 0), "uds_csr_create: NULL index array");
  UDS_REQUIRE(n_rows >= 0 && n_cols >= 0 && nnz >= 0 && n_rows < INT32_MAX && nnz < INT32_MAX,
              "uds_csr_create: sizes out of int32 range");
  UDS_REQUIRE(rowptr[0] == 0 && rowptr[n_rows] == nnz, "uds_csr_create: rowptr[0]=%d rowptr[n]=%d nnz=%lld",
              rowptr[0], rowptr[n_rows], (long long)nnz);
  int32_t max_deg = 0;
  for (int64_t r = 0; r < n_rows; ++r) {
    UDS_REQUIRE(rowptr[r + 1] >= rowptr[r], "uds_csr_create: rowptr decreases at row %lld", (long long)r);
    max_deg = std::max(max_deg, rowptr[r + 1] - rowptr[r]);
  }
  for (int64_t p = 0; p < nnz; ++p)
    UDS_REQUIRE(col[p] >= 0 && col[p] < n_cols, "uds_csr_create: col[%lld]=%d outside [0,%lld)",
                (long long)p, col[p], (long long)n_cols);
  uds_csr *c = new (std::nothrow) uds_csr;
  if (!c) return fail(UDS_ENOMEM, "uds_csr_create: host allocation failed");
  c->n_rows = n_rows;
  c->n_cols = n_cols;
  c->nnz = nnz;
  c->max_degree = max_deg;
  c->host.n_rows = n_rows;
  c->host.n_cols = n_cols;
  c->host.rowptr.assign(rowptr, rowptr + n_rows + 1);
  c->host.col.assign(col, col + nnz);
  constexpr int64_t ORDER_WINDOW = 1024;
// ... 976 lines not shown
}

static int gat_backward(const char *what, bool ex, const uds_csr_t *g, const uds_csr_t *gt, const int32_t *perm_t, const float *grad,
                        const float *hx, const float *s_self, const float *s_nbr, const float *a_self, const float *a_nbr,
                        const float *edge_mask, const float *coef, int64_t S, int64_t d, float *alpha_ws, float *de_ws, float *d_hx,
                        float *ds_self, float *ds_nbr, uds_stream_t stream) {
  const bool ptrs = perm_t && grad && hx && s_self && s_nbr && a_self && a_nbr && alpha_ws && de_ws && d_hx && ds_self && ds_nbr;
  if (int rc = gat_backward_check(what, ptrs, g, gt, false, 1, d, S, grad, hx, d_hx, a_self, a_nbr)) return rc;
  if (S == 0 || g->n_rows == 0) return UDS_OK;
  const int d4 = (int)(d / 4);
  hipStream_t st = static_cast<hipStream_t>(stream);
  uds::GatBwdRowsArgs ra{g->d_rowptr, g->d_col, grad, hx, s_self, s_nbr, alpha_ws, de_ws, ds_self,
                         (int)g->n_rows, d4, (int)S, uds::lanes_per_item(d4), g->nnz, coef, edge_mask};
  hipError_t e = ex ? uds::launch_gat_bwd_rows_ex(ra, st) : uds::launch_gat_bwd_rows(ra, st);
  if (e != hipSuccess) return fail(UDS_EHIP, "%s: row pass launch -> %s", what, hipGetErrorString(e));
  uds::GatBwdColsArgs ca{gt->d_rowptr, gt->d_col, perm_t, grad, alpha_ws, de_ws, ds_self, a_self, a_nbr, d_hx, ds_nbr,
                         (int)g->n_rows, d4, (int)S, g->nnz};
  e = uds::launch_gat_bwd_cols(ca, st);
  if (e != hipSuccess) return fail(UDS_EHIP, "%s: column pass launch -> %s", what, hipGetErrorString(e));
  return UDS_OK;
}

int uds_gat_backward(const uds_csr_t *g, const uds_csr_t *gt, const int32_t *perm_t, const float *grad, const float *hx,
                     const float *s_self, const float *s_nbr, const float *a_self, const float *a_nbr, int64_t S, int64_t d,
                     float *alpha_ws, float *de_ws, float *d_hx, float *ds_self, float *ds_nbr, uds_stream_t stream) {
  return uds_gat_backward_coef(g, gt, perm_t, grad, hx, s_self, s_nbr, a_self, a_nbr, nullptr, S, d, alpha_ws, de_ws, d_hx, ds_self, ds_nbr, stream);
}

int uds_gat_backward_coef(const uds_csr_t *g, const uds_csr_t *gt, const int32_t *perm_t, const float *grad, const float *hx,
                          const float *s_self, const float *s_nbr, const float *a_self, const float *a_nbr, const float *coef, int64_t S,
                          int64_t d, float *alpha_ws, float *de_ws, float *d_hx, float *ds_self, float *ds_nbr, uds_stream_t stream) {
  return gat_backward("uds_gat_backward", false, g, gt, perm_t, grad, hx, s_self, s_nbr, a_self, a_nbr, nullptr, coef, S, d, alpha_ws, de_ws, d_hx,
                      ds_self, ds_nbr, stream);
}

int uds_gat_backward_ex(const uds_csr_t *g, const uds_csr_t *gt, const int32_t *perm_t, const float *grad, const float *hx,
                        const float *s_self, const float *s_nbr, const float *a_self, const float *a_nbr, const float *edge_mask,
                        const float *coef, int64_t S, int64_t d, float *alpha_ws, float *de_ws, float *d_hx, float *ds_self,
                        float *ds_nbr, uds_stream_t stream) {
  return gat_backward("uds_gat_backward_ex", true, g, gt, perm_t, grad, hx, s_self, s_nbr, a_self, a_nbr, edge_mask, coef, S, d, alpha_ws, de_ws,
                      d_hx, ds_self, ds_nbr, stream);
}

int uds_gat_aggregate_heads(const uds_csr_t *g, const float *hx, const float *s_self, const float *s_nbr, const float *bias,
                            const float *edge_mask, const float *coef, int64_t S, int64_t H, int64_t C, int concat, int act,
                            float *out, float *alpha_out, uds_stream_t stream) {
  if (int rc = gat_aggregate_check("uds_gat_aggregate_heads", hx && s_self && s_nbr && out, g, true, H, C, S, act, hx, out, bias)) return rc;
  if (S == 0 || g->n_rows == 0) return UDS_OK;
  uds::GatHeadsArgs a{g->d_rowptr, g->d_col, g->d_order, hx, s_self, s_nbr, bias, edge_mask, coef, out, alpha_out,
                      (int)g->n_rows, (int)H, (int)(C / 4), act, (int)S, concat ? 0 : 1, g->nnz};
  return launched("uds_gat_aggregate_heads", uds::launch_gat_aggregate_heads(a, static_cast<hipStream_t>(stream)));
}

int uds_gat_backward_heads(const uds_csr_t *g, const uds_csr_t *gt, const int32_t *perm_t, const float *grad, const float *hx,
                           const float *s_self, const float *s_nbr, const float *a_self, const float *a_nbr,
                           const float *edge_mask, const float *coef, int64_t S, int64_t H, int64_t C, int concat,
                           float *alpha_ws, float *de_ws, float *d_hx, float *ds_self, float *ds_nbr, uds_stream_t stream) {
  const bool ptrs = perm_t && grad && hx && s_self && s_nbr && a_self && a_nbr && alpha_ws && de_ws && d_hx && ds_self && ds_nbr;
  if (int rc = gat_backward_check("uds_gat_backward_heads", ptrs, g, gt, true, H, C, S, grad, hx, d_hx, a_self, a_nbr)) return rc;
  if (S == 0 || g->n_rows == 0) return UDS_OK;
  const int c4 = (int)(C / 4);
  uds::GatBwdHeadsArgs a{g->d_rowptr, g->d_col, gt->d_rowptr, gt->d_col, perm_t, grad, hx, s_self, s_nbr, a_self, a_nbr, edge_mask, coef,
                         alpha_ws, de_ws, d_hx, ds_self, ds_nbr, (int)g->n_rows, (int)H, c4, (int)S, uds::lanes_per_item(c4),
                         concat ? 0 : 1, g->nnz};
  return launched("uds_gat_backward_heads", uds::launch_gat_bwd_heads(a, static_cast<hipStream_t>(stream)));
}

int uds_csr_sddmm(const uds_csr_t *csr, const float *a, const float *b, int64_t S, int64_t F, float *out, uds_stream_t stream) {
  UDS_REQUIRE(csr && a && b && out, "uds_csr_sddmm: NULL argument");
  UDS_REQUIRE(S >= 0 && F > 0 && F % 4 == 0, "uds_csr_sddmm: S=%lld F=%lld (F must be a positive multiple of 4)", (long long)S,
              (long long)F);
  UDS_REQUIRE(aligned16(a) && aligned16(b), "uds_csr_sddmm: a/b must be 16-byte aligned");
  if (csr->nnz == 0) return UDS_OK;
  const int f4 = (int)(F / 4);
  uds::SddmmArgs sa{csr->d_rowidx, csr->d_col, a, b, out, (int)csr->n_rows, (int)csr->n_cols, f4, (int)S, uds::lanes_per_item(f4),
                    csr->nnz};
  return launched("uds_csr_sddmm", uds::launch_csr_sddmm(sa, static_cast<hipStream_t>(stream)));
}

int64_t uds_wgrad_workspace_floats(int64_t rows, int64_t F, int64_t H, int with_bias) {
  const int mt = uds::wgrad_mt((int)(F + (with_bias ? 1 : 0))), nt = uds::wgrad_nt((int)H);
  if (!mt || !nt || rows <= 0) return 0;
  return (int64_t)uds::wgrad_grid(rows) * mt * 16 * nt * 16;
}

int uds_wgrad(const float *a, const float *g, int64_t B, int64_t T, int64_t R, int64_t F, int64_t H, int64_t shift, int with_bias,
              float *workspace, float *d_kernel, float *d_bias, uds_stream_t stream) {
  UDS_REQUIRE(a && g && workspace && d_kernel, "uds_wgrad: NULL argument");
  UDS_REQUIRE(!with_bias || d_bias, "uds_wgrad: with_bias needs d_bias");
  UDS_REQUIRE(B >= 0 && T > 0 && R > 0 && F > 0 && H > 0 && shift >= 0, "uds_wgrad: bad sizes");
  const int fr = (int)(F + (with_bias ? 1 : 0));
  const int mt = uds::wgrad_mt(fr), nt = uds::wgrad_nt((int)H);
  UDS_REQUIRE(mt && nt, "uds_wgrad: F=%lld (at most 128 rows incl. the bias row) or H=%lld (at most 64) not supported", (long long)F, (long long)H);
  UDS_REQUIRE(B * T * R < INT32_MAX, "uds_wgrad: %lld rows exceed the int32 row index", (long long)(B * T * R));
  hipStream_t st = static_cast<hipStream_t>(stream);
  const int64_t rows = B * T * R;
  if (rows == 0) {
    hipError_t e0 = hipMemsetAsync(d_kernel, 0, sizeof(float) * F * H, st);
    if (e0 == hipSuccess && with_bias) e0 = hipMemsetAsync(d_bias, 0, sizeof(float) * H, st);
    if (e0 != hipSuccess) return fail(UDS_EHIP, "uds_wgrad: memset -> %s", hipGetErrorString(e0));
    return UDS_OK;
  }
  const int grid = uds::wgrad_grid(rows);
  int64_t rpw = (rows + (int64_t)grid * 4 - 1) / ((int64_t)grid * 4);
  rpw = (rpw + 31) / 32 * 32;
  uds::WgradArgs wa{a, g, workspace, rows, (int)F, (int)H, with_bias ? (int)F : -1, (int)shift, (int)T, (int)R, (int)rpw};
  if (int rc = launched("uds_wgrad", uds::launch_wgrad(wa, mt, nt, grid, st))) return rc;
  hipLaunchKernelGGL(uds::k_wgrad_reduce, dim3((unsigned)((F * H + 15) / 16)), dim3(256), 0, st, workspace, grid, mt * 16, nt * 16,
                     (int)F, (int)H, d_kernel);
  if (with_bias)
    hipLaunchKernelGGL(uds::k_wgrad_reduce, dim3((unsigned)((H + 15) / 16)), dim3(256), 0, st, workspace + F * (nt * 16), grid,
                       mt * 16, nt * 16, 1, (int)H, d_bias);
  hipError_t e = hipGetLastError();
  if (e != hipSuccess) return fail(UDS_EHIP, "uds_wgrad: reduce launch -> %s", hipGetErrorString(e));
  return UDS_OK;
}

static int build_slot(uds_network *n, int fp, int fs) {
  uds_plan_slot &sl = n->slot[slot_index(fp, fs)];
  if (sl.built) return UDS_OK;
  sl.built = true;
  sl.fp = fp;
  sl.fs = fs;
  if ((fp == 128 || fs == 128) ? !plan_network128(n->adj->host, n->edge_adj->host, n->inc_n->host, n->inc_e->host, fp, fs, sl.plan, sl.lds_bytes)
                : !plan_network(n->adj->host, n->edge_adj->host, n->inc_n->host, n->inc_e->host, fp, fs, sl.plan, sl.lds_bytes, sl.blk_cap))
    return UDS_OK;
  hipError_t e;
  if ((e = hipMalloc(&sl.d_hdr, sizeof(int32_t) * sl.plan.hdr.size())) != hipSuccess ||
      (e = hipMalloc(&sl.d_pool, sizeof(int32_t) * sl.plan.pool.size())) != hipSuccess ||
      (e = hipMemcpy(sl.d_hdr, sl.plan.hdr.data(), sizeof(int32_t) * sl.plan.hdr.size(), hipMemcpyHostToDevice)) != hipSuccess ||
      (e = hipMemcpy(sl.d_pool, sl.plan.pool.data(), sizeof(int32_t) * sl.plan.pool.size(), hipMemcpyHostToDevice)) != hipSuccess)
    return fail(UDS_ENOMEM, "tile plan upload -> %s", hipGetErrorString(e));
  auto upload_blocks = [&](const std::vector<int32_t> &hdr, int n_tiles, int32_t **dst) -> hipError_t {
    if (fp == 128 || fs == 128) return hipSuccess;
    std::vector<int32_t> bl;
    uds::build_ell_blocks(hdr, sl.plan.pool, n_tiles, sl.blk_cap, bl);
    hipError_t e2 = hipMalloc(dst, sizeof(int32_t) * bl.size());
    if (e2 != hipSuccess) return e2;
    return hipMemcpy(*dst, bl.data(), sizeof(int32_t) * bl.size(), hipMemcpyHostToDevice);
  };
  if ((e = upload_blocks(sl.plan.hdr, sl.plan.n_tiles, &sl.d_blocks)) != hipSuccess)
    return fail(UDS_ENOMEM, "tile block upload -> %s", hipGetErrorString(e));
  for (int side = 0; side < 2; ++side) {
    std::vector<int32_t> hs;
    for (int t = 0; t < sl.plan.n_tiles; ++t)
      if (sl.plan.hdr[(size_t)t * uds::TILE_HDR_INTS + 6] == side)
        hs.insert(hs.end(), sl.plan.hdr.begin() + (size_t)t * uds::TILE_HDR_INTS, sl.plan.hdr.begin() + (size_t)(t + 1) * uds::TILE_HDR_INTS);
    if ((e = hipMalloc(&sl.d_hdr_side[side], sizeof(int32_t) * std::max<size_t>(hs.size(), 1))) != hipSuccess ||
        (!hs.empty() && (e = hipMemcpy(sl.d_hdr_side[side], hs.data(), sizeof(int32_t) * hs.size(), hipMemcpyHostToDevice)) != hipSuccess))
      return fail(UDS_ENOMEM, "tile plan upload -> %s", hipGetErrorString(e));
    if ((e = upload_blocks(hs, (int)(hs.size() / uds::TILE_HDR_INTS), &sl.d_blocks_side[side])) != hipSuccess)
      return fail(UDS_ENOMEM, "tile block upload -> %s", hipGetErrorString(e));
  }
  sl.ok = true;
  return UDS_OK;
}

int uds_network_prepare(uds_network_t *net, int64_t fx, int64_t fe) {
  UDS_REQUIRE(net != nullptr, "uds_network_prepare: NULL network");
  if (net->adj->n_rows == 0 || net->edge_adj->n_rows == 0) return UDS_OK;
  if (fx == 128 && (fe == 128 || fe == 64)) {
    int rc = build_slot(net, 128, (int)fe);
    if (rc == UDS_OK && fe == 64) rc = build_slot(net, 64, 128);
    return rc;
  }
  if (!((fx == 64 || fx == 96) && (fe == 64 || fe == 96))) return UDS_OK;
  int rc = build_slot(net, (int)fx, (int)fe);
  if (rc == UDS_OK) rc = build_slot(net, (int)fe, (int)fx);
  return rc;
}

int uds_network_create(const uds_csr_t *adj, const uds_csr_t *edge_adj, const uds_csr_t *inc_n, const uds_csr_t *inc_e,
                       uds_network_t **out) {
  UDS_REQUIRE(out != nullptr, "uds_network_create: out is NULL");
  *out = nullptr;
  UDS_REQUIRE(adj && edge_adj && inc_n && inc_e, "uds_network_create: NULL pattern");
  const int64_t N = adj->n_rows, E = edge_adj->n_rows;
  UDS_REQUIRE(adj->n_cols == N && edge_adj->n_cols == E, "uds_network_create: adjacency patterns must be square");
  UDS_REQUIRE(inc_n->n_rows == N && inc_n->n_cols == E && inc_e->n_rows == E && inc_e->n_cols == N,
              "uds_network_create: incidence shapes (%lld x %lld), (%lld x %lld) do not match N=%lld E=%lld",
              (long long)inc_n->n_rows, (long long)inc_n->n_cols, (long long)inc_e->n_rows, (long long)inc_e->n_cols,
              (long long)N, (long long)E);
  uds_network *n = new (std::nothrow) uds_network;
  if (!n) return fail(UDS_ENOMEM, "uds_network_create: host allocation failed");
  n->adj = adj;
  n->edge_adj = edge_adj;
  n->inc_n = inc_n;
  n->inc_e = inc_e;
  if (N > 0 && E > 0) {
    int rc = build_slot(n, 64, 64);
    if (rc != UDS_OK) {
      uds_network_destroy(n);
      return rc;
    }
  }
  *out = n;
  return UDS_OK;
}

int uds_network_destroy(uds_network_t *net) {
  if (!net) return UDS_OK;
  for (uds_plan_slot &sl : net->slot) {
    hipFree(sl.d_hdr);
    hipFree(sl.d_pool);
    hipFree(sl.d_hdr_side[0]);
    hipFree(sl.d_hdr_side[1]);
    hipFree(sl.d_blocks);
    hipFree(sl.d_blocks_side[0]);
    hipFree(sl.d_blocks_side[1]);
  }
  delete net;
  return UDS_OK;
}

int uds_network_plan_info(const uds_network_t *net, int32_t *info8) {
  UDS_REQUIRE(net && info8, "uds_network_plan_info: NULL argument");
  const uds_plan_slot &sl = net->slot[0];
  info8[0] = (sl.ok ? 1 : 0) | ((net->slot[1].ok && net->slot[2].ok) ? 2 : 0) | (net->slot[3].ok ? 4 : 0) | (net->slot[4].ok ? 8 : 0) |
             ((net->slot[5].ok && net->slot[6].ok) ? 16 : 0);
  info8[1] = sl.plan.side[0].n_tiles;
  info8[2] = sl.plan.side[1].n_tiles;
  info8[3] = sl.plan.p_cap;
  info8[4] = sl.plan.q_cap;
  info8[5] = sl.blk_cap ? sl.blk_cap : sl.plan.meta_cap;
  info8[6] = (int32_t)sl.lds_bytes;
  info8[7] = sl.plan.t_max[0] * 1000 + sl.plan.t_max[1];
  return UDS_OK;
}

int uds_tile_plan_create(const int32_t *adj_rowptr, const int32_t *adj_col, const int32_t *eadj_rowptr, const int32_t *eadj_col,
                         const int32_t *incn_rowptr, const int32_t *incn_col, const int32_t *ince_rowptr, const int32_t *ince_col,
                         int64_t n_node, int64_t n_edge, int32_t t_node, int32_t t_link, int32_t p_limit, int32_t q_limit,
                         uds_tile_plan_t **out) {
  UDS_REQUIRE(out != nullptr, "uds_tile_plan_create: out is NULL");
  *out = nullptr;
  UDS_REQUIRE(adj_rowptr && adj_col && eadj_rowptr && eadj_col && incn_rowptr && ince_rowptr, "uds_tile_plan_create: NULL array");
  UDS_REQUIRE(n_node > 0 && n_edge > 0 && t_node >= 1 && t_link >= 1, "uds_tile_plan_create: bad sizes");
  auto mk = [](const int32_t *rp, const int32_t *c, int64_t r, int64_t cc) {
    uds::HostCsr h;
    h.n_rows = r;
    h.n_cols = cc;
    h.rowptr.assign(rp, rp + r + 1);
    h.col.assign(c, c + rp[r]);
    return h;
  };
  uds_tile_plan *tp = new (std::nothrow) uds_tile_plan;
  if (!tp) return fail(UDS_ENOMEM, "uds_tile_plan_create: host allocation failed");
  tp->plan = uds::build_network_plan(mk(adj_rowptr, adj_col, n_node, n_node), mk(eadj_rowptr, eadj_col, n_edge, n_edge),
                                     mk(incn_rowptr, incn_col, n_node, n_edge), mk(ince_rowptr, ince_col, n_edge, n_node),
                                     t_node, t_link, p_limit, q_limit);
  *out = tp;
  return UDS_OK;
}

int uds_tile_plan_destroy(uds_tile_plan_t *tp) {
  delete tp;
  return UDS_OK;
}

int uds_tile_plan_sizes(const uds_tile_plan_t *tp, int64_t *n_tiles, int64_t *pool_len, int32_t *caps3) {
  UDS_REQUIRE(tp != nullptr, "uds_tile_plan_sizes: NULL plan");
  if (n_tiles) *n_tiles = tp->plan.n_tiles;
  if (pool_len) *pool_len = (int64_t)tp->plan.pool.size();
  if (caps3) {
    caps3[0] = tp->plan.p_cap;
    caps3[1] = tp->plan.q_cap;
    caps3[2] = tp->plan.meta_cap;
  }
  return UDS_OK;
}

int uds_tile_plan_copy(const uds_tile_plan_t *tp, int32_t *hdr_out, int32_t *pool_out) {
  UDS_REQUIRE(tp && hdr_out && pool_out, "uds_tile_plan_copy: NULL argument");
  std::memcpy(hdr_out, tp->plan.hdr.data(), sizeof(int32_t) * tp->plan.hdr.size());
  std::memcpy(pool_out, tp->plan.pool.data(), sizeof(int32_t) * tp->plan.pool.size());
  return UDS_OK;
}

int uds_tile_plan_blocks(const uds_tile_plan_t *tp, int32_t *blocks_out, int64_t *stride_out) {
  UDS_REQUIRE(tp != nullptr, "uds_tile_plan_blocks: NULL plan");
  const int cap = uds::ell_block_cap(tp->plan.hdr, tp->plan.pool, tp->plan.n_tiles);
  UDS_REQUIRE(cap >= 0, "uds_tile_plan_blocks: a tile has more than 255 primary / 256 secondary rows (byte-wide local indices)");
  if (stride_out) *stride_out = cap;
  if (!blocks_out) return UDS_OK;
  std::vector<int32_t> bl;
  uds::build_ell_blocks(tp->plan.hdr, tp->plan.pool, tp->plan.n_tiles, cap, bl);
  std::memcpy(blocks_out, bl.data(), sizeof(int32_t) * (size_t)cap * tp->plan.n_tiles);
  return UDS_OK;
}

int64_t uds_spatial_workspace_floats(const uds_network_t *net, int64_t S, int64_t h, int64_t d) {
  if (!net) return 0;
  const int64_t N = net->adj->n_rows, E = net->edge_adj->n_rows;
  return PACKED_WEIGHT_FLOATS + S * 2 * (N + E) * h + align4(S * N * (d + 2)) + align4(S * E * (d + 2));
}


int64_t uds_spatial_packed_bytes(void) { return PACKED_WEIGHT_FLOATS * 4; }

int uds_spatial_pack_weights(const uds_spatial_params_t *p, int64_t fx, int64_t fe, int64_t h, int64_t d, void *packed_out,
                             uds_stream_t stream) {
  UDS_REQUIRE(p && packed_out && p->xe_k && p->ex_k && p->gx_k && p->ge_k, "uds_spatial_pack_weights: NULL argument");
  const bool wide = h == uds::F128_H && d == uds::F128_D && fx == 128 && (fe == 128 || fe == 64);
  UDS_REQUIRE(wide || (h == uds::FUSED_H && d == uds::FUSED_D && (fx == 64 || fx == 96) && (fe == 64 || fe == 96)),
              "uds_spatial_pack_weights: the fused kernels take h=32, d=64, fx, fe in {64, 96} or h=64, d=128, fx=128, fe in {64, 128} (got h=%lld d=%lld "
              "fx=%lld fe=%lld)", (long long)h, (long long)d, (long long)fx, (long long)fe);
  UDS_REQUIRE(aligned16(packed_out), "uds_spatial_pack_weights: output must be 16-byte aligned");
  hipStream_t st = static_cast<hipStream_t>(stream);
  uint4 *wq = reinterpret_cast<uint4 *>(packed_out);
  hipError_t he;
  const int o_small = wide ? 2048 : 768, o_big = wide ? 6144 : 2048;
  if ((he = pack_weights(p->xe_k, (int)fe, (int)h, wq, st)) != hipSuccess ||
      (he = pack_weights(p->gx_k, (int)(fx + h), (int)d, wq + o_small, st)) != hipSuccess ||
      (he = pack_weights(p->ex_k, (int)fx, (int)h, wq + o_small + o_big, st)) != hipSuccess ||
      (he = pack_weights(p->ge_k, (int)(fe + h), (int)d, wq + 2 * o_small + o_big, st)) != hipSuccess)
    return fail(UDS_EHIP, "uds_spatial_pack_weights: launch -> %s", hipGetErrorString(he));
  if (!wide && fx == 64 && fe == 64) {
    const int total = (int)((fx + h) / 16) * (int)(d / 32) * 64;
    hipLaunchKernelGGL(uds::k_pack_weight_frags32, dim3((total + 255) / 256), dim3(256), 0, st, p->gx_k, (int)(fx + h), (int)d, wq + WS_BIG32_OFF);
    hipLaunchKernelGGL(uds::k_pack_weight_frags32, dim3((total + 255) / 256), dim3(256), 0, st, p->ge_k, (int)(fe + h), (int)d, wq + WS_BIG32_OFF + WS_BIG32_LEN);
    const int ts = (int)(fe / 16) * (int)(h / 32) * 64;
    hipLaunchKernelGGL(uds::k_pack_weight_frags32, dim3((ts + 255) / 256), dim3(256), 0, st, p->xe_k, (int)fe, (int)h, wq + WS_SMALL32_OFF);
    hipLaunchKernelGGL(uds::k_pack_weight_frags32, dim3((ts + 255) / 256), dim3(256), 0, st, p->ex_k, (int)fx, (int)h, wq + WS_SMALL32_OFF + WS_SMALL32_LEN);
    return launched("uds_spatial_pack_weights", hipGetLastError());
  }
  return UDS_OK;
}

int uds_spatial_layer_forward(const uds_network_t *net, const uds_spatial_params_t *p, const float *x, int64_t fx,
                              const float *e, int64_t fe, int64_t S, int64_t h, int64_t d, int act, int flags, float *ws,
                              float *out_x, float *out_e, uds_stream_t stream) {
  return uds_spatial_layer_forward_split(net, p, x, fx, nullptr, 0, e, fe, nullptr, 0, S, h, d, act, flags, ws, out_x, out_e, stream);
}

static int spatial_forward_impl(const uds_network_t *net, const uds_spatial_params_t *p, const float *x, int64_t fxa,
                                const float *xb, int64_t fxb, const float *e, int64_t fea, const float *eb, int64_t feb,
                                const float *rem_x, const float *rem_e, int64_t S, int64_t h, int64_t d, int act, int flags,
                                float *ws, float *out_x, float *out_e, uds_stream_t stream);

int uds_spatial_layer_forward_split(const uds_network_t *net, const uds_spatial_params_t *p, const float *x, int64_t fxa,
                                    const float *xb, int64_t fxb, const float *e, int64_t fea, const float *eb, int64_t feb,
                                    int64_t S, int64_t h, int64_t d, int act, int flags, float *ws, float *out_x, float *out_e,
                                    uds_stream_t stream) {
  return spatial_forward_impl(net, p, x, fxa, xb, fxb, e, fea, eb, feb, nullptr, nullptr, S, h, d, act, flags, ws, out_x, out_e, stream);
}

int uds_spatial_layer_forward_rem(const uds_network_t *net, const uds_spatial_params_t *p, const float *x, int64_t fx,
                                  const float *e, int64_t fe, const float *rem_x, const float *rem_e, int64_t S, int64_t h,
                                  int64_t d, int act, int flags, float *ws, float *out_x, float *out_e, uds_stream_t stream) {
  UDS_REQUIRE(rem_x && rem_e, "uds_spatial_layer_forward_rem: NULL remainder");
  UDS_REQUIRE(aligned16(rem_x) && aligned16(rem_e), "uds_spatial_layer_forward_rem: rem_x / rem_e must be 16-byte aligned");
  return spatial_forward_impl(net, p, x, fx, nullptr, 0, e, fe, nullptr, 0, rem_x, rem_e, S, h, d, act, flags | UDS_FLAG_REQUIRE_FUSED, ws,
                              out_x, out_e, stream);
}

static int spatial_forward_impl(const uds_network_t *net, const uds_spatial_params_t *p, const float *x, int64_t fxa,
                                const float *xb, int64_t fxb, const float *e, int64_t fea, const float *eb, int64_t feb,
                                const float *rem_x, const float *rem_e, int64_t S, int64_t h, int64_t d, int act, int flags,
                                float *ws, float *out_x, float *out_e, uds_stream_t stream) {
  UDS_REQUIRE(net && p && x && e && ws && out_x && out_e, "uds_spatial_layer_forward: NULL argument");
  UDS_REQUIRE((xb != nullptr) == (fxb > 0) && (eb != nullptr) == (feb > 0), "uds_spatial_layer_forward_split: xb/fxb or eb/feb disagree");
  UDS_REQUIRE((!xb || (fxa == 64 && fxb == 32)) && (!eb || (fea == 64 && feb == 32)),
              "uds_spatial_layer_forward_split: a split input must be 64 + 32 columns (got %lld+%lld, %lld+%lld)", (long long)fxa,
              (long long)fxb, (long long)fea, (long long)feb);
  UDS_REQUIRE(aligned16(xb) && aligned16(eb), "uds_spatial_layer_forward_split: xb/eb must be 16-byte aligned");
  const int64_t fx = fxa + fxb, fe = fea + feb;
  if (xb || eb) flags |= UDS_FLAG_REQUIRE_FUSED;
  UDS_REQUIRE(p->xe_k && p->ex_k && p->ne_n_val && p->ne_e_val && p->gx_k && p->gx_as && p->gx_an && p->ge_k &&
                  p->ge_as && p->ge_an,
              "uds_spatial_layer_forward: NULL parameter tensor");
  UDS_REQUIRE(h > 0 && h % 4 == 0 && d > 0 && d % 4 == 0, "uds_spatial_layer_forward: h=%lld d=%lld must be multiples of 4",
              (long long)h, (long long)d);
  UDS_REQUIRE(act >= UDS_ACT_LINEAR && act <= UDS_ACT_HARD_SIGMOID, "uds_spatial_layer_forward: unknown activation %d", act);
  UDS_REQUIRE(out_x != x && out_e != e, "uds_spatial_layer_forward: outputs must not alias inputs");
  UDS_REQUIRE(aligned16(x) && aligned16(e) && aligned16(ws) && aligned16(out_x) && aligned16(out_e),
              "uds_spatial_layer_forward: x/e/workspace/outputs must be 16-byte aligned");
  const int64_t N = net->adj->n_rows, E = net->edge_adj->n_rows;
  hipStream_t st = static_cast<hipStream_t>(stream);
  if (S == 0) return UDS_OK;

  if (h == uds::F128_H && d == uds::F128_D && fx == 128 && (fe == 128 || fe == 64) && !xb && !eb && !(flags & UDS_FLAG_EXACT_FP32) &&
      net->slot[slot_index(128, (int)fe)].ok && net->slot[slot_index((int)fe, 128)].ok) {
    UDS_REQUIRE(aligned16(p->xe_b) && aligned16(p->ex_b) && aligned16(p->gx_as) && aligned16(p->gx_an) && aligned16(p->gx_b) &&
                    aligned16(p->ge_as) && aligned16(p->ge_an) && aligned16(p->ge_b),
                "uds_spatial_layer_forward: bias / attention vectors must be 16-byte aligned");
    const uint4 *wq = reinterpret_cast<const uint4 *>(p->packed);
    if (!wq) {
      int rc = uds_spatial_pack_weights(p, fx, fe, h, d, ws, stream);
      if (rc != UDS_OK) return rc;
      wq = reinterpret_cast<const uint4 *>(ws);
    } else {
      UDS_REQUIRE(aligned16(wq), "uds_spatial_layer_forward: packed weights must be 16-byte aligned");
    }
    uds::FusedArgs a;
    a.blocks = nullptr;
    a.side[0] = uds::FusedSide{x, e, nullptr, nullptr, out_x, wq, wq + 2048, nullptr, nullptr, p->xe_b, p->gx_as, p->gx_an, p->gx_b, p->ne_n_val, (int)N, (int)E, rem_x};
    a.side[1] = uds::FusedSide{e, x, nullptr, nullptr, out_e, wq + 8192, wq + 10240, nullptr, nullptr, p->ex_b, p->ge_as, p->ge_an, p->ge_b, p->ne_e_val, (int)E, (int)N, rem_e};
    a.S = (int)S;
    a.act = act;
    a.dbg = nullptr;
#ifdef UDS_PHASE_TIMING
    a.dbg = reinterpret_cast<unsigned long long *>(ws + PACKED_WEIGHT_FLOATS);
#endif
    auto launch_side = [&](const uds_plan_slot &u, int side, auto FP_, auto FS_) {
      a.hdr = side < 0 ? u.d_hdr : u.d_hdr_side[side];
      a.pool = u.d_pool;
      a.n_tiles = side < 0 ? u.plan.n_tiles : u.plan.side[side].n_tiles;
      a.p_cap = u.plan.p_cap;
      a.q_cap = u.plan.q_cap;
      a.meta_cap = u.plan.meta_cap;
      a.side_mask = side < 0 ? 3 : (1 << side);
      if ((rem_x || rem_e) && a.p_cap > 64) return hipErrorInvalidValue;
      const int64_t chunk = pick_chunk(S, a.n_tiles);
      a.chunk = (int)chunk;
      const int grid = (int)(((S + chunk - 1) / chunk) * a.n_tiles);
      return launch_fused128<decltype(FP_)::value, decltype(FS_)::value>(a, grid, u.lds_bytes, st);
    };
    using I64 = std::integral_constant<int, 64>;
    using I128 = std::integral_constant<int, 128>;
    hipError_t he;
    if (fe == 128) {
      he = launch_side(net->slot[4], -1, I128{}, I128{});
    } else {
      he = launch_side(net->slot[5], 0, I128{}, I64{});
      if (he == hipSuccess) he = launch_side(net->slot[6], 1, I64{}, I128{});
    }
    if (he != hipSuccess) return fail(UDS_EHIP, "uds_spatial_layer_forward: fused d=128 launch -> %s", hipGetErrorString(he));
    return UDS_OK;
  }
  UDS_REQUIRE((!rem_x && !rem_e) || (h == uds::FUSED_H && d == uds::FUSED_D && fxa == 64 && fea == 64),
              "uds_spatial_layer_forward_rem: the remainder goes into the d = 128 fused kernel or the 64-wide d = 64 one (fx=%lld fe=%lld h=%lld d=%lld, plan %d)",
              (long long)fxa, (long long)fea, (long long)h, (long long)d, (int)(net->slot[4].ok));
  const bool shape_ok = h == uds::FUSED_H && d == uds::FUSED_D && (fx == 64 || fx == 96) && (fe == 64 || fe == 96) &&
                        std::max(N, E) * 384 < ((int64_t)1 << 31);
  const uds_plan_slot &sl = net->slot[slot_index((int)fx, (int)fe)];
  const uds_plan_slot &sl_link = net->slot[slot_index((int)fe, (int)fx)];
  if (flags & UDS_FLAG_REQUIRE_FUSED)
    UDS_REQUIRE(sl.ok && sl_link.ok && shape_ok && !(flags & UDS_FLAG_EXACT_FP32),
                "uds_spatial_layer_forward: fused kernel unavailable (plan %d, fx=%lld fe=%lld h=%lld d=%lld)", (int)sl.ok,
                (long long)fx, (long long)fe, (long long)h, (long long)d);
  if (sl.ok && sl_link.ok && shape_ok && !(flags & UDS_FLAG_EXACT_FP32)) {
    UDS_REQUIRE(aligned16(p->xe_b) && aligned16(p->ex_b) && aligned16(p->gx_as) && aligned16(p->gx_an) && aligned16(p->gx_b) &&
                    aligned16(p->ge_as) && aligned16(p->ge_an) && aligned16(p->ge_b),
                "uds_spatial_layer_forward: bias / attention vectors must be 16-byte aligned");
    hipError_t he;
    const uint4 *wq = reinterpret_cast<const uint4 *>(p->packed);
    if (!wq) {
      int rc = uds_spatial_pack_weights(p, fx, fe, h, d, ws, stream);
      if (rc != UDS_OK) return rc;
      wq = reinterpret_cast<const uint4 *>(ws);
    } else {
      UDS_REQUIRE(aligned16(wq), "uds_spatial_layer_forward: packed weights must be 16-byte aligned");
    }
    const uint4 *w_small_n = wq, *w_big_n = wq + 768, *w_small_e = wq + 768 + 2048, *w_big_e = wq + 2 * 768 + 2048;
    uds::FusedArgs a;
    a.blocks = nullptr;
    const bool has32 = fx == 64 && fe == 64;
    a.side[0] = uds::FusedSide{x, e, xb, eb, out_x, w_small_n, w_big_n, has32 ? wq + WS_BIG32_OFF : nullptr, has32 ? wq + WS_SMALL32_OFF : nullptr, p->xe_b, p->gx_as, p->gx_an, p->gx_b, p->ne_n_val, (int)N, (int)E, rem_x};
    a.side[1] = uds::FusedSide{e, x, eb, xb, out_e, w_small_e, w_big_e, has32 ? wq + WS_BIG32_OFF + WS_BIG32_LEN : nullptr, has32 ? wq + WS_SMALL32_OFF + WS_SMALL32_LEN : nullptr, p->ex_b, p->ge_as, p->ge_an, p->ge_b, p->ne_e_val, (int)E, (int)N, rem_e};
    int64_t lds_need = 0;
    auto use_plan = [&](const uds_plan_slot &u, int side) {
      a.hdr = side < 0 ? u.d_hdr : u.d_hdr_side[side];
      a.pool = u.d_pool;
      a.n_tiles = side < 0 ? u.plan.n_tiles : u.plan.side[side].n_tiles;
      a.p_cap = u.plan.p_cap;
      a.q_cap = u.plan.q_cap;
      a.meta_cap = u.blk_cap;
      a.blocks = side < 0 ? u.d_blocks : u.d_blocks_side[side];
      lds_need = u.lds_bytes;
    };
    use_plan(sl, -1);
    a.S = (int)S;
    a.act = act;
    a.dbg = nullptr;
#ifdef UDS_PHASE_TIMING
    a.dbg = reinterpret_cast<unsigned long long *>(ws + PACKED_WEIGHT_FLOATS);
#endif
    auto set_chunk = [&](int64_t working_tiles) {
      int64_t chunk = pick_chunk(S, working_tiles);
#ifdef UDS_KNOBS
      if (const char *ov = std::getenv("UDS_CHUNK")) chunk = std::max<int64_t>(1, std::min<int64_t>(S, std::atoll(ov)));
#endif
      a.chunk = (int)chunk;
      return (int)(((S + chunk - 1) / chunk) * a.n_tiles);
    };
    if (fx == fe) {
      a.side_mask = 3;
      const int grid = set_chunk(a.n_tiles);
      const int64_t ws_lds = uds::fused_ws_lds_bytes(a.p_cap, a.q_cap, a.meta_cap);
      bool ws = fx == 64 && !xb && !eb && ws_lds <= FUSED_LDS_BUDGET && a.p_cap <= 128 && a.q_cap <= 256;
#ifdef UDS_KNOBS
      if (std::getenv("UDS_NO_WS")) ws = false;
#endif
      UDS_REQUIRE(ws || (!rem_x && !rem_e), "uds_spatial_layer_forward_rem: the wave-specialised d = 64 kernel cannot take this network's plan (p_cap %d, q_cap %d, %lld B of LDS)",
                  a.p_cap, a.q_cap, (long long)ws_lds);
      if (ws) he = launch_fused_ws(a, grid, ws_lds, st);
      else he = (fx == 64) ? launch_fused<64, 64>(a, grid, lds_need, st) : launch_fused<96, 96>(a, grid, lds_need, st);
    } else {
      a.side_mask = 1;
      use_plan(sl, 0);
      int grid = set_chunk(a.n_tiles);
      he = (fx == 64) ? launch_fused<64, 96>(a, grid, lds_need, st) : launch_fused<96, 64>(a, grid, lds_need, st);
      if (he == hipSuccess) {
        a.side_mask = 2;
        use_plan(sl_link, 1);
        grid = set_chunk(a.n_tiles);
        he = (fe == 64) ? launch_fused<64, 96>(a, grid, lds_need, st) : launch_fused<96, 64>(a, grid, lds_need, st);
      }
    }
    if (he != hipSuccess) return fail(UDS_EHIP, "uds_spatial_layer_forward: fused launch -> %s", hipGetErrorString(he));
    return UDS_OK;
  }

  float *base = ws + PACKED_WEIGHT_FLOATS;
  float *x_e = base;
  float *e_x = x_e + S * E * h;
  float *agg_n = e_x + S * N * h;
  float *agg_e = agg_n + S * N * h;
  float *gat_ws_n = agg_e + S * E * h;
  float *gat_ws_e = gat_ws_n + align4(S * N * (d + 2));
  int rc;
  if ((rc = uds_dense_act(e, fe, nullptr, 0, S * E, p->xe_k, p->xe_b, h, act, nullptr, nullptr, x_e, nullptr, nullptr, stream))) return rc;
  if ((rc = uds_dense_act(x, fx, nullptr, 0, S * N, p->ex_k, p->ex_b, h, act, nullptr, nullptr, e_x, nullptr, nullptr, stream))) return rc;
  if ((rc = uds_csr_spmm(net->inc_n, p->ne_n_val, x_e, S, h, nullptr, UDS_ACT_LINEAR, agg_n, stream))) return rc;
  if ((rc = uds_csr_spmm(net->inc_e, p->ne_e_val, e_x, S, h, nullptr, UDS_ACT_LINEAR, agg_e, stream))) return rc;
  if ((rc = uds_gat_forward(net->adj, x, fx, agg_n, h, S, p->gx_k, p->gx_as, p->gx_an, p->gx_b, d, act, gat_ws_n, out_x, stream))) return rc;
  if ((rc = uds_gat_forward(net->edge_adj, e, fe, agg_e, h, S, p->ge_k, p->ge_as, p->ge_an, p->ge_b, d, act, gat_ws_e, out_e, stream))) return rc;
  return UDS_OK;
}

}
```

### include/uds_hip.h

```cpp
#ifndef UDS_HIP_H
#define UDS_HIP_H

#include <stdint.h>

#ifdef __cplusplus
extern "C" {
#endif

#define UDS_ABI_VERSION 22

enum {
  UDS_OK = 0,
  UDS_EINVAL = -22,
  UDS_ENOMEM = -12,
  UDS_EHIP = -5,
  UDS_ENOSYS = -38
};

enum {
  UDS_ACT_LINEAR = 0,
  UDS_ACT_RELU = 1,
  UDS_ACT_TANH = 2,
  UDS_ACT_SIGMOID = 3,
  UDS_ACT_HARD_SIGMOID = 4
// ... 111 lines not shown
typedef struct {
  const void *a_packed;
  const float *a_bias;
  const void *h_packed[5];
  const float *h_bias[5];
  const void *f_packed;
  const float *f_bias;
  int32_t n_a, act_a, n_hidden, act_h, act_f;
} uds_heads_t;
int uds_dense_cumsum_heads(const float *x, int64_t B, int64_t T, int64_t R, const void *packed, const float *bias,
                           const float *res, int act, const uds_heads_t *heads, float *out, uds_stream_t stream);

typedef struct {
  const void *packed[3];
  const float *bias[3];
  int32_t n_layers, act;
} uds_conv_stack_t;
int uds_conv_stack_plan(int64_t B, int64_t T, int64_t R, int n_layers, int64_t *n_seg, int64_t *seg_len, int64_t *halo);
int uds_conv_stack_forward(const float *x, int64_t B, int64_t T, int64_t R, const uds_conv_stack_t *layers, int64_t n_seg,
                           float *out, uds_stream_t stream);

int uds_cumsum_act(const float *x, const float *res, int64_t B, int64_t T, int64_t R, int64_t F, int act,
                   float *out, uds_stream_t stream);

int uds_attn_sum_pool(const float *x, const float *k, int64_t B, int64_t R, int64_t F, float *out, uds_stream_t stream);

int uds_attn_sum_pool_pair(const float *x, int64_t Rx, const float *e, int64_t Re, const float *k, int64_t B, int64_t F, float *out,
                           float *stat, uds_stream_t stream);

int uds_attn_sum_pool_backward(const float *x, int64_t Rx, const float *e, int64_t Re, const float *k, const float *out,
                               const float *stat, const float *grad, int64_t B, int64_t F, float *dx, float *de, float *dk_ws,
                               float *dk, uds_stream_t stream);

int uds_dropout(const float *x, int64_t n, float rate, uint64_t seed, uint64_t offset, float *out, uds_stream_t stream);

int uds_flow_balance(const uds_csr_t *inc_n, const float *sign, const float *flow, int64_t S,
                     const float *scale_in, const float *scale_out, float *q_in, float *q_out,
                     uds_stream_t stream);

int uds_roll_update(const uds_csr_t *inc_n, const float *sign, const float *span_e, const float *mini_e,
                    const float *scale_in, const float *scale_out, const float *y, int64_t cy, const float *ey,
                    int64_t ce, const float *b, int64_t B, int64_t so, int64_t T, int flood, float *x, float *ex,
                    float *preds, uds_stream_t stream);

typedef struct uds_tail {
  int32_t N, E, cy, ce, n_act, b_channels;
  int32_t edge_fusion, tide, has_offset, act, pump_override, any_pump, if_flood;
  float depth_gate, epsilon;
  const float *is_outfall, *hmin, *hmax, *area_eps, *ps, *pump_in, *pump_out, *ny_in, *ny_out, *scale_in, *scale_out;
  const float *span_y, *mini_y;
  const float *offset, *pump, *pump_mask, *pump_den, *ehmax, *from_ok;
  const float *span_e, *mini_e;
  const int32_t *from_node;
  const int32_t *act_link, *act_in, *act_out;
  const int32_t *link_node;
  const float *link_sign;
  const int32_t *al_ptr, *al_idx, *ai_ptr, *ai_idx, *ao_ptr, *ao_idx;
} uds_tail_t;

int uds_predict_tail(const uds_csr_t *inc_n, const float *sign, const uds_tail_t *p, const float *y, const float *ey,
                     const float *a, const float *b_norm, const float *runoff, const float *h0, int64_t B, int64_t T,
                     float *out_y, float *out_ey, uds_stream_t stream);

int64_t uds_predict_tail_workspace_floats(int64_t N, int64_t E, int64_t B, int64_t T);

int uds_predict_tail_backward(const uds_csr_t *inc_n, const float *sign, const uds_tail_t *p, const float *y,
                              const float *ey, const float *a, const float *b_norm, const float *runoff,
                              const float *h0, int64_t B, int64_t T, const float *g_out_y, const float *g_out_ey,
                              float *dy, float *dey, float *da, float *dh0, float *workspace, uds_stream_t stream);

int uds_fit_tail(const uds_csr_t *inc_n, const float *sign, const uds_tail_t *p, const float *y, const float *ey,
                 const float *a, const float *b_norm, const float *y_true, const float *ey_true, const float *nwei,
                 const float *poswei, const float *ewei, const float *qw_den, const float *span_b, const float *mini_b,
                 int64_t B, int64_t T, int64_t cyt, int balance, float *out_y, float *out_ey, float *loss_sums,
                 float *workspace, uds_stream_t stream);

int64_t uds_fit_tail_workspace_floats(int64_t N, int64_t E, int64_t B, int64_t T);

int uds_fit_tail_backward(const uds_csr_t *inc_n, const float *sign, const uds_tail_t *p, const float *y, const float *ey,
                          const float *a, const float *b_norm, const float *y_true, const float *ey_true,
                          const float *nwei, const float *poswei, const float *ewei, const float *qw_den,
                          const float *span_b, const float *mini_b, int64_t B, int64_t T, int64_t cyt, int balance,
                          const float *g_loss, const float *g_out_y, const float *g_out_ey, float *dy, float *dey,
                          float *workspace, uds_stream_t stream);

int64_t uds_gat_workspace_floats(int64_t n, int64_t S, int64_t d);

int uds_gat_forward(const uds_csr_t *graph, const float *xa, int64_t fa, const float *xb,
                    int64_t fb, int64_t S, const float *W, const float *a_self,
                    const float *a_nbr, const float *bias, int64_t d, int act, float *workspace,
                    float *out, uds_stream_t stream);

int uds_gat_aggregate(const uds_csr_t *graph, const float *hx, const float *s_self, const float *s_nbr,
                      const float *bias, int64_t S, int64_t d, int act, float *out, uds_stream_t stream);


int uds_gat_aggregate_masked(const uds_csr_t *graph, const float *hx, const float *s_self, const float *s_nbr,
                             const float *bias, const float *edge_mask, int64_t S, int64_t d, int act, float *out,
                             uds_stream_t stream);

int uds_gat_backward(const uds_csr_t *graph, const uds_csr_t *graph_t, const int32_t *perm_t, const float *grad,
                     const float *hx, const float *s_self, const float *s_nbr, const float *a_self,
                     const float *a_nbr, int64_t S, int64_t d, float *alpha_ws, float *de_ws, float *d_hx,
                     float *ds_self, float *ds_nbr, uds_stream_t stream);

int uds_gat_aggregate_coef(const uds_csr_t *g, const float *hx, const float *s_self, const float *s_nbr, const float *bias,
                           const float *coef, int64_t S, int64_t d, int act, float *out, uds_stream_t stream);
int uds_gat_backward_coef(const uds_csr_t *g, const uds_csr_t *gt, const int32_t *perm_t, const float *grad, const float *hx,
                          const float *s_self, const float *s_nbr, const float *a_self, const float *a_nbr, const float *coef,
                          int64_t S, int64_t d, float *alpha_ws, float *de_ws, float *d_hx, float *ds_self, float *ds_nbr,
                          uds_stream_t stream);

int uds_gat_aggregate_ex(const uds_csr_t *g, const float *hx, const float *s_self, const float *s_nbr, const float *bias,
                         const float *edge_mask, const float *coef, int64_t S, int64_t d, int act, float *out,
                         uds_stream_t stream);
int uds_gat_backward_ex(const uds_csr_t *g, const uds_csr_t *gt, const int32_t *perm_t, const float *grad, const float *hx,
                        const float *s_self, const float *s_nbr, const float *a_self, const float *a_nbr,
                        const float *edge_mask, const float *coef, int64_t S, int64_t d, float *alpha_ws, float *de_ws,
                        float *d_hx, float *ds_self, float *ds_nbr, uds_stream_t stream);

int uds_gat_aggregate_heads(const uds_csr_t *g, const float *hx, const float *s_self, const float *s_nbr, const float *bias,
                            const float *edge_mask, const float *coef, int64_t S, int64_t H, int64_t C, int concat, int act,
                            float *out, float *alpha_out, uds_stream_t stream);
int uds_gat_backward_heads(const uds_csr_t *g, const uds_csr_t *gt, const int32_t *perm_t, const float *grad, const float *hx,
                           const float *s_self, const float *s_nbr, const float *a_self, const float *a_nbr,
                           const float *edge_mask, const float *coef, int64_t S, int64_t H, int64_t C, int concat,
                           float *alpha_ws, float *de_ws, float *d_hx, float *ds_self, float *ds_nbr, uds_stream_t stream);

int uds_csr_sddmm(const uds_csr_t *csr, const float *a, const float *b, int64_t S, int64_t F, float *out,
                  uds_stream_t stream);

int64_t uds_wgrad_workspace_floats(int64_t rows, int64_t F, int64_t H, int with_bias);
int uds_wgrad(const float *a, const float *g, int64_t B, int64_t T, int64_t R, int64_t F, int64_t H, int64_t shift,
              int with_bias, float *workspace, float *d_kernel, float *d_bias, uds_stream_t stream);

typedef struct uds_network uds_network_t;

int uds_network_create(const uds_csr_t *adj, const uds_csr_t *edge_adj, const uds_csr_t *inc_n,
                       const uds_csr_t *inc_e, uds_network_t **out);
int uds_network_destroy(uds_network_t *net);
int uds_network_prepare(uds_network_t *net, int64_t fx, int64_t fe);
int uds_network_plan_info(const uds_network_t *net, int32_t *info8);

typedef struct uds_tile_plan uds_tile_plan_t;
int uds_tile_plan_create(const int32_t *adj_rowptr, const int32_t *adj_col, const int32_t *eadj_rowptr,
                         const int32_t *eadj_col, const int32_t *incn_rowptr, const int32_t *incn_col,
                         const int32_t *ince_rowptr, const int32_t *ince_col, int64_t n_node,
                         int64_t n_edge, int32_t t_node, int32_t t_link, int32_t p_limit,
                         int32_t q_limit, uds_tile_plan_t **out);
int uds_tile_plan_destroy(uds_tile_plan_t *plan);
int uds_tile_plan_sizes(const uds_tile_plan_t *plan, int64_t *n_tiles, int64_t *pool_len, int32_t *caps3);
int uds_tile_plan_copy(const uds_tile_plan_t *plan, int32_t *hdr_out, int32_t *pool_out);
int uds_tile_plan_blocks(const uds_tile_plan_t *plan, int32_t *blocks_out, int64_t *stride_out);

typedef struct uds_spatial_params {
  const float *xe_k, *xe_b;
  const float *ex_k, *ex_b;
  const float *ne_n_val;
  const float *ne_e_val;
  const float *gx_k, *gx_as, *gx_an, *gx_b;
  const float *ge_k, *ge_as, *ge_an, *ge_b;
  const void *packed;
} uds_spatial_params_t;

int64_t uds_spatial_packed_bytes(void);
int uds_spatial_pack_weights(const uds_spatial_params_t *params, int64_t fx, int64_t fe, int64_t h, int64_t d,
                             void *packed_out, uds_stream_t stream);

enum {
  UDS_FLAG_EXACT_FP32 = 1,
  UDS_FLAG_REQUIRE_FUSED = 2
};

int64_t uds_spatial_workspace_floats(const uds_network_t *net, int64_t S, int64_t h, int64_t d);

int uds_spatial_layer_forward(const uds_network_t *net, const uds_spatial_params_t *params,
                              const float *x, int64_t fx, const float *e, int64_t fe, int64_t S,
                              int64_t h, int64_t d, int act, int flags, float *workspace,
                              float *out_x, float *out_e, uds_stream_t stream);

int uds_spatial_layer_forward_split(const uds_network_t *net, const uds_spatial_params_t *params, const float *xa,
                                    int64_t fxa, const float *xb, int64_t fxb, const float *ea, int64_t fea,
                                    const float *eb, int64_t feb, int64_t S, int64_t h, int64_t d, int act, int flags,
                                    float *workspace, float *out_x, float *out_e, uds_stream_t stream);

int uds_spatial_layer_forward_rem(const uds_network_t *net, const uds_spatial_params_t *params, const float *x, int64_t fx,
                                  const float *e, int64_t fe, const float *rem_x, const float *rem_e, int64_t S, int64_t h,
                                  int64_t d, int act, int flags, float *workspace, float *out_x, float *out_e,
                                  uds_stream_t stream);

#ifdef __cplusplus
}
#endif
#endif
```

Before: 292,900.

## Balance X-team wave work with a planner-built per-tile octet/block assignment table

```diff
diff --git a/gnn_uds_amd/_lib.py b/gnn_uds_amd/_lib.py
--- a/gnn_uds_amd/_lib.py
+++ b/gnn_uds_amd/_lib.py
@@ -8,7 +8,7 @@
 LIB_PATH = os.environ.get('UDS_LIB_PATH') or os.path.join(_HERE, 'libuds_hip.so')
 
 ABI_VERSION = 22
-FLAG_EXACT_FP32, FLAG_REQUIRE_FUSED = 1, 2
+FLAG_EXACT_FP32, FLAG_REQUIRE_FUSED, FLAG_ONE_CHUNK = 1, 2, 4
 PRECISION_FLAGS = {'bf16x3': 0, 'fp32': FLAG_EXACT_FP32}
 
 ACT = {None: 0, 'linear': 0, 'relu': 1, 'tanh': 2, 'sigmoid': 3, 'hard_sigmoid': 4}
@@ -110,6 +110,10 @@
     'uds_tile_plan_sizes': (_c_int, [_c_ptr, ctypes.POINTER(_c_i64), ctypes.POINTER(_c_i64), _c_ptr]),
     'uds_tile_plan_copy': (_c_int, [_c_ptr, _c_ptr, _c_ptr]),
     'uds_tile_plan_blocks': (_c_int, [_c_ptr, _c_ptr, ctypes.POINTER(_c_i64)]),
+    'uds_tile_plan_xteam': (_c_int, [_c_ptr, _c_ptr]),
+    'uds_tile_plan_xteam_load': (_c_int, [_c_ptr, _c_ptr, _c_ptr]),
+    'uds_network_set_xteam': (_c_int, [_c_ptr, _c_ptr]),
+    'uds_network_get_xteam': (_c_int, [_c_ptr, _c_ptr, _c_ptr]),
     'uds_roll_update': (_c_int, [_c_ptr] * 7 + [_c_i64, _c_ptr, _c_i64, _c_ptr, _c_i64, _c_i64, _c_i64, _c_int, _c_ptr, _c_ptr, _c_ptr, _c_ptr]),
     'uds_predict_tail': (_c_int, [_c_ptr] * 9 + [_c_i64, _c_i64, _c_ptr, _c_ptr, _c_ptr]),
     'uds_predict_tail_workspace_floats': (_c_i64, [_c_i64, _c_i64, _c_i64, _c_i64]),
@@ -313,13 +317,28 @@
         out['t_node'], out['t_link'] = out['t_code'] // 1000, out['t_code'] % 1000
         return out
 
+    def xteam(self):
+        info = self.plan_info()
+        n = info['node_tiles'] + info['link_tiles']
+        units, table = np.zeros((n, 2), dtype=np.int32), np.zeros((n, 2), dtype=np.int32)
+        _check(load().uds_network_get_xteam(self._h, units.ctypes.data, table.ctypes.data), 'uds_network_get_xteam')
+        return units, table
+
+    def set_xteam(self, table=None):
+        if table is not None:
+            table = np.ascontiguousarray(table, dtype=np.int32)
+            n = self.plan_info()
+            if table.shape != (n['node_tiles'] + n['link_tiles'], 2):
+                raise ValueError(f'set_xteam: table of shape {table.shape} for {n["node_tiles"] + n["link_tiles"]} tiles')
+        _check(load().uds_network_set_xteam(self.ptr, None if table is None else table.ctypes.data), 'uds_network_set_xteam')
+
     def __del__(self):
         h, self._h = getattr(self, '_h', None), None
         if h is not None and _lib is not None:
             _lib.uds_network_destroy(h)
 
 
-def tile_plan(graph, t_node=48, t_link=48, p_limit=0, q_limit=0, blocks=False):
+def tile_plan(graph, t_node=48, t_link=48, p_limit=0, q_limit=0, blocks=False, xteam=False):
     lib = load()
     arrs = []
     for c in (graph.adj, graph.edge_adj, graph.inc_n, graph.inc_e):
@@ -340,9 +359,20 @@
             if lib.uds_tile_plan_blocks(h, None, ctypes.byref(stride)) == 0:
                 blk = np.zeros((nt.value, stride.value), dtype=np.int32)
                 _check(lib.uds_tile_plan_blocks(h, blk.ctypes.data, ctypes.byref(stride)), 'uds_tile_plan_blocks')
+        xt = None
+        if xteam is not False:
+            xt = np.zeros((nt.value, 2), dtype=np.int32)
+            load4 = np.zeros((nt.value, 4), dtype=np.int32)
+            if xteam is True:
+                _check(lib.uds_tile_plan_xteam(h, xt.ctypes.data), 'uds_tile_plan_xteam')
+            else:
+                xt[...] = np.asarray(xteam, dtype=np.int32).reshape(nt.value, 2)
+            _check(lib.uds_tile_plan_xteam_load(h, xt.ctypes.data, load4.ctypes.data), 'uds_tile_plan_xteam_load')
     finally:
         lib.uds_tile_plan_destroy(h)
     out = dict(p_cap=int(caps[0]), q_cap=int(caps[1]), meta_cap=int(caps[2]))
+    if xt is not None:
+        out['xteam'], out['xteam_load'] = xt, load4
     if blocks:
         out['blocks'] = blk
     return hdr, pool, out
diff --git a/gnn_uds_amd/csrc/kernels_fused.hpp b/gnn_uds_amd/csrc/kernels_fused.hpp
--- a/gnn_uds_amd/csrc/kernels_fused.hpp
+++ b/gnn_uds_amd/csrc/kernels_fused.hpp
@@ -34,6 +34,7 @@
   FusedSide side[2];
   const int32_t *hdr, *pool;
   const int32_t *blocks;
+  const int32_t *xteam;
   int n_tiles, S, chunk, p_cap, q_cap, meta_cap, act, side_mask;
   unsigned long long *dbg;
 };
diff --git a/gnn_uds_amd/csrc/kernels_fused_ws.hpp b/gnn_uds_amd/csrc/kernels_fused_ws.hpp
--- a/gnn_uds_amd/csrc/kernels_fused_ws.hpp
+++ b/gnn_uds_amd/csrc/kernels_fused_ws.hpp
@@ -71,6 +71,7 @@
   const int chunk_id = w / a.n_tiles;
   const int s_begin = chunk_id * a.chunk;
   const int s_end = min(a.S, (chunk_id + 1) * a.chunk);
+  const int xt_lane = a.xteam[2 * tile + (tid & 1)];
   const int sd = __builtin_amdgcn_readfirstlane(a.hdr[tile * TILE_HDR_INTS + 6]);
   if (!((a.side_mask >> sd) & 1)) return;
   const FusedSide &S_ = a.side[sd];
@@ -94,6 +95,7 @@
     attn[2 * FUSED_D + FUSED_H + tid] = S_.b_out ? S_.b_out[tid] : 0.f;
   }
   __syncthreads();
+  const unsigned xt_oct = (unsigned)__builtin_amdgcn_readlane(xt_lane, 0), xt_blk = (unsigned)__builtin_amdgcn_readlane(xt_lane, 1);
   const int n_own = __builtin_amdgcn_readfirstlane(smem[0]), n_prim = __builtin_amdgcn_readfirstlane(smem[1]),
             n_sec = __builtin_amdgcn_readfirstlane(smem[2]), flags = __builtin_amdgcn_readfirstlane(smem[3]),
             n_ovf = __builtin_amdgcn_readfirstlane(smem[4]), n_adj = __builtin_amdgcn_readfirstlane(smem[5]),
@@ -276,7 +278,24 @@
     __builtin_amdgcn_s_setprio(WS_XPRIO);
     typedef float f32x16 __attribute__((ext_vector_type(16)));
     constexpr int KS32 = FS / 16, SJ32 = (8 + NX - 1) / NX;
+    static_assert(NX == XT_WAVES && U == XT_MAX_OCT && SJ32 == XT_MAX_BLK && WS_OCT_WD == XT_OCT_WD, "the planner deals for this team shape");
     const int n32 = lane & 31, hf = lane >> 5;
+    int oc[U], bk[SJ32];
+    {
+      unsigned long long mo = xt_oct ^ (0x55555555u * (unsigned)xw), mb = xt_blk ^ (0x5555u * (unsigned)xw);
+      mo = ~(mo | (mo >> 1)) & 0x55555555ull & ((1ull << (2 * ((n_own + 7) >> 3))) - 1);
+      mb = ~(mb | (mb >> 1)) & 0x5555ull & ((1ull << (2 * ((n_sec + 31) >> 5))) - 1);
+#pragma unroll
+      for (int u = 0; u < U; ++u) {
+        oc[u] = __builtin_amdgcn_readfirstlane(__builtin_ctzll(mo | (1ull << 32)) >> 1);
+        mo &= mo - 1;
+      }
+#pragma unroll
+      for (int j = 0; j < SJ32; ++j) {
+        bk[j] = __builtin_amdgcn_readfirstlane(__builtin_ctzll(mb | (1ull << 16)) >> 1);
+        mb &= mb - 1;
+      }
+    }
     bf16x8 w1h[KS32], w1l[KS32];
 #pragma unroll
     for (int t = 0; t < KS32; ++t) {
@@ -285,7 +304,7 @@
     }
     unsigned srow[SJ32];
 #pragma unroll
-    for (int j = 0; j < SJ32; ++j) srow[j] = ((unsigned)sec_ids[min((xw + NX * j) * 32 + n32, n_sec - 1)] * FS + 8u * hf) * 4u;
+    for (int j = 0; j < SJ32; ++j) srow[j] = ((unsigned)sec_ids[min(bk[j] * 32 + n32, n_sec - 1)] * FS + 8u * hf) * 4u;
     f32x4 sp[SJ32][2 * KS32];
     auto load_sec_at = [&](const float *base) __attribute__((always_inline)) {
       static_for<SJ32>([&](auto j_) {
@@ -308,7 +327,7 @@
     int n_st = 0;
 #pragma unroll
     for (int u = 0; u < U; ++u) {
-      const int i = 8 * (NX * u + xw) + ro;
+      const int i = 8 * oc[u] + ro;
       const int ic = min(i, n_own - 1);
       int dmx;
       if (flags & ELL_FLAG_LONG_ROWS) {
@@ -333,7 +352,7 @@
         p3_pk[u][k2] = pk;
       }
       p3_jb4 |= (i < n_own ? (unsigned)adj_b[i * ELL_ADJ + c8] : 0xFFu) << (8 * u);
-      if (8 * (NX * u + xw) < n_own) n_st += 2;
+      if (8 * oc[u] < n_own) n_st += 2;
     }
     const float *bias_l = attn + 2 * FUSED_D + FUSED_H + 4 * c8;
     __builtin_amdgcn_s_waitcnt(0x0F70);
@@ -342,7 +361,8 @@
       float *secw = sec + buf * sec_buf;
       static_for<SJ32>([&](auto j_) {
         constexpr int j = decltype(j_)::value;
-        const int blk = xw + NX * j;
+        int blk = bk[j];
+        asm volatile("" : "+s"(blk));
         if (blk * 32 < n_sec) {
           f32x16 acc;
 #pragma unroll
@@ -398,6 +418,8 @@
       asm volatile("" : "+s"(d0), "+s"(d1), "+s"(d2), "+s"(d3));
       const int e3 = d3, e2 = max(e3, d2), e1 = max(e2, d1), e0 = max(e1, d0);
       if (e0 == 0) return;
+      int ou[U] = {oc[0], oc[1], oc[2], oc[3]};
+      asm volatile("" : "+s"(ou[0]), "+s"(ou[1]), "+s"(ou[2]), "+s"(ou[3]));
 
       float ss[U], lg0[U], lg1[U], w0[U], w1[U], den[U];
       bool ok[U], has0[U], has1[U];
@@ -405,9 +427,9 @@
       int joff1[U];
 #pragma unroll
       for (int u = 0; u < U; ++u) {
-        ok[u] = 8 * (NX * u + xw) + ro < n_own;
+        ok[u] = 8 * ou[u] + ro < n_own;
         jb0[u] = (p3_jb4 >> (8 * u)) & 0xFFu;
-        ss[u] = ssr[8 * (NX * u + xw) + ro];
+        ss[u] = ssr[8 * ou[u] + ro];
       }
 #pragma unroll
       for (int u = 0; u < U; ++u) has0[u] = ok[u] && jb0[u] != 0xFFu;
@@ -430,7 +452,7 @@
         if (ext) {
           float m1[U];
 #pragma unroll
-          for (int u = 0; u < U; ++u) jb1[u] = adj_b[(8 * (NX * u + xw) + ro) * ELL_ADJ + 8 + c8];
+          for (int u = 0; u < U; ++u) jb1[u] = adj_b[(8 * ou[u] + ro) * ELL_ADJ + 8 + c8];
           asm volatile("" : "+v"(jb1[0]), "+v"(jb1[1]), "+v"(jb1[2]), "+v"(jb1[3]));
 #pragma unroll
           for (int u = 0; u < U; ++u) sn[u] = snr[jb1[u]];
@@ -532,7 +554,7 @@
       } else {
 #pragma unroll
         for (int u = 0; u < U; ++u) {
-          const int i = 8 * (NX * u + xw) + ro;
+          const int i = 8 * ou[u] + ro;
           const int b0 = i < n_own ? adj_ptr[i] : 0;
           const int dg = i < n_own ? adj_ptr[i + 1] - b0 : 0;
           float mx = -INFINITY;
@@ -555,7 +577,7 @@
       f32x4 bo0 = *reinterpret_cast<const f32x4 *>(bias_l + 32 * hf8), bo1 = *reinterpret_cast<const f32x4 *>(bias_l + 32 - 32 * hf8);
       int pid[U];
 #pragma unroll
-      for (int u = 0; u < U; ++u) pid[u] = prim_ids[8 * (NX * u + xw) + ro];
+      for (int u = 0; u < U; ++u) pid[u] = prim_ids[8 * ou[u] + ro];
       asm volatile("" : "+v"(pid[0]), "+v"(pid[1]), "+v"(pid[2]), "+v"(pid[3]), "+v"(bo0), "+v"(bo1));
       float *out_s = out_snap + (4 * c8 + 32 * hf8);
       const int o1_off = 32 - 64 * hf8;
diff --git a/gnn_uds_amd/csrc/tile_plan.hpp b/gnn_uds_amd/csrc/tile_plan.hpp
--- a/gnn_uds_amd/csrc/tile_plan.hpp
+++ b/gnn_uds_amd/csrc/tile_plan.hpp
@@ -431,6 +431,127 @@
   }
 }
 
+constexpr int XT_WAVES = 4, XT_MAX_OCT = 4, XT_MAX_BLK = 2, XT_OCT_WD = 4;
+constexpr int XT_C_BLOCK = 1450;
+constexpr int XT_C_P3 = 1800;
+constexpr int XT_C_OCT = 150;
+constexpr int XT_C_STEP = 600;
+constexpr int XT_C_EXT = 600;
+constexpr int XT_C_LONG = 40;
+
+struct XteamItems {
+  int n_oct = 0, n_blk = 0;
+  int cost[16] = {};
+  bool ext[16] = {};
+};
+inline bool xteam_fits(const int32_t *hd) { return hd[0] <= 8 * XT_WAVES * XT_MAX_OCT && hd[2] <= 32 * XT_WAVES * XT_MAX_BLK; }
+inline XteamItems xteam_items(const TileView &v) {
+  XteamItems it;
+  it.n_oct = (v.n_own + 7) / 8;
+  it.n_blk = (v.n_sec + 31) / 32;
+  bool long_rows = false;
+  for (int i = 0; i < v.n_own; ++i) long_rows |= v.adj_ptr[i + 1] - v.adj_ptr[i] > ELL_ADJ;
+  for (int o = 0; o < it.n_oct && o < 16; ++o) {
+    int dmax = 0, dsum = 0;
+    for (int i = 8 * o; i < std::min(8 * o + 8, v.n_own); ++i) {
+      const int d = v.adj_ptr[i + 1] - v.adj_ptr[i];
+      dmax = std::max(dmax, d);
+      dsum += d;
+    }
+    if (long_rows) {
+      it.cost[o] = XT_C_OCT + XT_C_LONG * dsum;
+    } else {
+      const int s0 = (std::min(dmax, 8) + XT_OCT_WD - 1) / XT_OCT_WD, s1 = (std::max(dmax, 8) - 8 + XT_OCT_WD - 1) / XT_OCT_WD;
+      it.cost[o] = XT_C_OCT + XT_C_STEP * (s0 + s1);
+      it.ext[o] = dmax > 8;
+    }
+  }
+  return it;
+}
+inline bool xteam_valid(int n_oct, int n_blk, uint32_t w_oct, uint32_t w_blk) {
+  if (n_oct > XT_WAVES * XT_MAX_OCT || n_blk > XT_WAVES * XT_MAX_BLK) return false;
+  if (n_oct < 16 && (w_oct >> (2 * n_oct))) return false;
+  if ((uint64_t)w_blk >> (2 * n_blk)) return false;
+  int co[XT_WAVES] = {}, cb[XT_WAVES] = {};
+  for (int o = 0; o < n_oct; ++o) ++co[(w_oct >> (2 * o)) & 3];
+  for (int b = 0; b < n_blk; ++b) ++cb[(w_blk >> (2 * b)) & 3];
+  for (int w = 0; w < XT_WAVES; ++w)
+    if (co[w] > XT_MAX_OCT || cb[w] > XT_MAX_BLK) return false;
+  return true;
+}
+inline void xteam_load(const XteamItems &it, uint32_t w_oct, uint32_t w_blk, int (&load)[XT_WAVES]) {
+  bool any[XT_WAVES] = {}, ext[XT_WAVES] = {};
+  for (int w = 0; w < XT_WAVES; ++w) load[w] = 0;
+  for (int b = 0; b < it.n_blk; ++b) load[(w_blk >> (2 * b)) & 3] += XT_C_BLOCK;
+  for (int o = 0; o < it.n_oct; ++o) {
+    const int w = (w_oct >> (2 * o)) & 3;
+    load[w] += it.cost[o];
+    any[w] = true;
+    ext[w] |= it.ext[o];
+  }
+  for (int w = 0; w < XT_WAVES; ++w) load[w] += (any[w] ? XT_C_P3 : 0) + (ext[w] ? XT_C_EXT : 0);
+}
+inline int xteam_max_load(const XteamItems &it, uint32_t w_oct, uint32_t w_blk) {
+  int load[XT_WAVES];
+  xteam_load(it, w_oct, w_blk, load);
+  return *std::max_element(load, load + XT_WAVES);
+}
+inline void xteam_round_robin(int n_oct, int n_blk, uint32_t &w_oct, uint32_t &w_blk) {
+  w_oct = w_blk = 0;
+  for (int o = 0; o < n_oct; ++o) w_oct |= (uint32_t)(o % XT_WAVES) << (2 * o);
+  for (int b = 0; b < n_blk; ++b) w_blk |= (uint32_t)(b % XT_WAVES) << (2 * b);
+}
+inline void xteam_deal(const XteamItems &it, uint32_t &w_oct, uint32_t &w_blk) {
+  struct Unit { int cost, kind, idx; };
+  std::vector<Unit> units;
+  for (int o = 0; o < it.n_oct; ++o) units.push_back({it.cost[o], 0, o});
+  for (int b = 0; b < it.n_blk; ++b) units.push_back({XT_C_BLOCK, 1, b});
+  std::stable_sort(units.begin(), units.end(), [](const Unit &x, const Unit &y) {
+    return x.cost != y.cost ? x.cost > y.cost : (x.kind != y.kind ? x.kind < y.kind : x.idx < y.idx);
+  });
+  int load[XT_WAVES] = {}, co[XT_WAVES] = {}, cb[XT_WAVES] = {};
+  bool ext[XT_WAVES] = {};
+  uint32_t go = 0, gb = 0;
+  for (const Unit &u : units) {
+    int best = -1, best_load = 0;
+    for (int w = 0; w < XT_WAVES; ++w) {
+      if (u.kind == 0 ? co[w] >= XT_MAX_OCT : cb[w] >= XT_MAX_BLK) continue;
+      int l = load[w] + u.cost;
+      if (u.kind == 0) l += (co[w] == 0 ? XT_C_P3 : 0) + (it.ext[u.idx] && !ext[w] ? XT_C_EXT : 0);
+      if (best < 0 || l < best_load) {
+        best = w;
+        best_load = l;
+      }
+    }
+    load[best] = best_load;
+    if (u.kind == 0) {
+      ++co[best];
+      ext[best] |= it.ext[u.idx];
+      go |= (uint32_t)best << (2 * u.idx);
+    } else {
+      ++cb[best];
+      gb |= (uint32_t)best << (2 * u.idx);
+    }
+  }
+  xteam_round_robin(it.n_oct, it.n_blk, w_oct, w_blk);
+  if (xteam_max_load(it, go, gb) < xteam_max_load(it, w_oct, w_blk)) {
+    w_oct = go;
+    w_blk = gb;
+  }
+}
+inline bool build_xteam(const std::vector<int32_t> &hdr, const std::vector<int32_t> &pool, int n_tiles, std::vector<int32_t> &out) {
+  out.assign(std::max<size_t>(2 * (size_t)n_tiles, 2), 0);
+  for (int t = 0; t < n_tiles; ++t) {
+    const int32_t *hd = hdr.data() + (size_t)t * TILE_HDR_INTS;
+    if (!xteam_fits(hd)) return false;
+    uint32_t wo, wb;
+    xteam_deal(xteam_items(tile_view(hd, pool.data())), wo, wb);
+    out[2 * (size_t)t] = (int32_t)wo;
+    out[2 * (size_t)t + 1] = (int32_t)wb;
+  }
+  return true;
+}
+
 inline int64_t fused_lds_bytes(int p_cap, int q_cap, int meta_cap, int h, int d, int fp, int fs) {
   const int64_t weights = 16 * 64 * 2 * ((int64_t)(fs / 32) * (h / 16) + (int64_t)((fp + h) / 32) * (d / 16));
   const int64_t stage = std::max<int64_t>(4 * ((int64_t)q_cap * fs + (int64_t)p_cap * fp), weights);
diff --git a/gnn_uds_amd/csrc/uds_hip.hip b/gnn_uds_amd/csrc/uds_hip.hip
--- a/gnn_uds_amd/csrc/uds_hip.hip
+++ b/gnn_uds_amd/csrc/uds_hip.hip
@@ -88,6 +88,8 @@
   int32_t *d_hdr_side[2] = {nullptr, nullptr};
   int32_t *d_blocks = nullptr, *d_blocks_side[2] = {nullptr, nullptr};
   int blk_cap = 0;
+  std::vector<int32_t> xteam_plan, xteam_now;
+  int32_t *d_xteam = nullptr;
   int64_t lds_bytes = 0;
 };
 
@@ -1370,6 +1372,12 @@
     if ((e = upload_blocks(hs, (int)(hs.size() / uds::TILE_HDR_INTS), &sl.d_blocks_side[side])) != hipSuccess)
       return fail(UDS_ENOMEM, "tile block upload -> %s", hipGetErrorString(e));
   }
+  if (fp == 64 && fs == 64 && uds::build_xteam(sl.plan.hdr, sl.plan.pool, sl.plan.n_tiles, sl.xteam_plan)) {
+    if ((e = hipMalloc(&sl.d_xteam, sizeof(int32_t) * sl.xteam_plan.size())) != hipSuccess ||
+        (e = hipMemcpy(sl.d_xteam, sl.xteam_plan.data(), sizeof(int32_t) * sl.xteam_plan.size(), hipMemcpyHostToDevice)) != hipSuccess)
+      return fail(UDS_ENOMEM, "X-team table upload -> %s", hipGetErrorString(e));
+    sl.xteam_now = sl.xteam_plan;
+  }
   sl.ok = true;
   return UDS_OK;
 }
@@ -1426,6 +1434,7 @@
     hipFree(sl.d_blocks);
     hipFree(sl.d_blocks_side[0]);
     hipFree(sl.d_blocks_side[1]);
+    hipFree(sl.d_xteam);
   }
   delete net;
   return UDS_OK;
@@ -1504,6 +1513,76 @@
   std::vector<int32_t> bl;
   uds::build_ell_blocks(tp->plan.hdr, tp->plan.pool, tp->plan.n_tiles, cap, bl);
   std::memcpy(blocks_out, bl.data(), sizeof(int32_t) * (size_t)cap * tp->plan.n_tiles);
+  return UDS_OK;
+}
+
+static int check_xteam(const uds::NetworkPlan &plan, const int32_t *table, const char *who) {
+  for (int t = 0; t < plan.n_tiles; ++t) {
+    const int32_t *hd = plan.hdr.data() + (size_t)t * uds::TILE_HDR_INTS;
+    UDS_REQUIRE(uds::xteam_fits(hd), "%s: tile %d has %d own / %d secondary rows, more than the X team holds (128 / 256)", who, t, hd[0], hd[2]);
+    if (table)
+      UDS_REQUIRE(uds::xteam_valid((hd[0] + 7) / 8, (hd[2] + 31) / 32, (uint32_t)table[2 * t], (uint32_t)table[2 * t + 1]),
+                  "%s: tile %d: words %08x %08x are not a partition of its %d octets and %d blocks with at most %d octets and %d blocks per wave",
+                  who, t, (unsigned)table[2 * t], (unsigned)table[2 * t + 1], (hd[0] + 7) / 8, (hd[2] + 31) / 32, uds::XT_MAX_OCT, uds::XT_MAX_BLK);
+  }
+  return UDS_OK;
+}
+
+int uds_tile_plan_xteam(const uds_tile_plan_t *tp, int32_t *out) {
+  UDS_REQUIRE(tp && out, "uds_tile_plan_xteam: NULL argument");
+  if (int rc = check_xteam(tp->plan, nullptr, "uds_tile_plan_xteam")) return rc;
+  std::vector<int32_t> tb;
+  uds::build_xteam(tp->plan.hdr, tp->plan.pool, tp->plan.n_tiles, tb);
+  std::memcpy(out, tb.data(), sizeof(int32_t) * 2 * (size_t)tp->plan.n_tiles);
+  return UDS_OK;
+}
+
+int uds_tile_plan_xteam_load(const uds_tile_plan_t *tp, const int32_t *table, int32_t *load_out) {
+  UDS_REQUIRE(tp && load_out, "uds_tile_plan_xteam_load: NULL argument");
+  if (int rc = check_xteam(tp->plan, table, "uds_tile_plan_xteam_load")) return rc;
+  std::vector<int32_t> tb;
+  if (!table) {
+    uds::build_xteam(tp->plan.hdr, tp->plan.pool, tp->plan.n_tiles, tb);
+    table = tb.data();
+  }
+  for (int t = 0; t < tp->plan.n_tiles; ++t) {
+    int load[uds::XT_WAVES];
+    uds::xteam_load(uds::xteam_items(uds::tile_view(tp->plan.hdr.data() + (size_t)t * uds::TILE_HDR_INTS, tp->plan.pool.data())),
+                    (uint32_t)table[2 * t], (uint32_t)table[2 * t + 1], load);
+    std::copy(load, load + uds::XT_WAVES, load_out + (size_t)uds::XT_WAVES * t);
+  }
+  return UDS_OK;
+}
+
+int uds_network_set_xteam(uds_network_t *net, const int32_t *table) {
+  UDS_REQUIRE(net != nullptr, "uds_network_set_xteam: NULL network");
+  uds_plan_slot &sl = net->slot[0];
+  UDS_REQUIRE(sl.ok && sl.d_xteam, "uds_network_set_xteam: the network has no plan for the wave-specialised kernel");
+  if (int rc = check_xteam(sl.plan, table, "uds_network_set_xteam")) return rc;
+  const int32_t *src = table ? table : sl.xteam_plan.data();
+  hipError_t e;
+  if ((e = hipDeviceSynchronize()) != hipSuccess ||
+      (e = hipMemcpy(sl.d_xteam, src, sizeof(int32_t) * 2 * (size_t)sl.plan.n_tiles, hipMemcpyHostToDevice)) != hipSuccess)
+    return fail(UDS_EHIP, "uds_network_set_xteam: upload -> %s", hipGetErrorString(e));
+  sl.xteam_now.assign(src, src + 2 * (size_t)sl.plan.n_tiles);
+  return UDS_OK;
+}
+
+int uds_network_get_xteam(const uds_network_t *net, int32_t *units_out, int32_t *table_out) {
+  UDS_REQUIRE(net != nullptr, "uds_network_get_xteam: NULL network");
+  const uds_plan_slot &sl = net->slot[0];
+  UDS_REQUIRE(sl.ok && sl.d_xteam, "uds_network_get_xteam: the network has no plan for the wave-specialised kernel");
+  for (int t = 0; t < sl.plan.n_tiles; ++t) {
+    const int32_t *hd = sl.plan.hdr.data() + (size_t)t * uds::TILE_HDR_INTS;
+    if (units_out) {
+      units_out[2 * t] = (hd[0] + 7) / 8;
+      units_out[2 * t + 1] = (hd[2] + 31) / 32;
+    }
+    if (table_out) {
+      table_out[2 * t] = sl.xteam_now[2 * (size_t)t];
+      table_out[2 * t + 1] = sl.xteam_now[2 * (size_t)t + 1];
+    }
+  }
   return UDS_OK;
 }
 
@@ -1612,6 +1691,7 @@
     }
     uds::FusedArgs a;
     a.blocks = nullptr;
+    a.xteam = nullptr;
     a.side[0] = uds::FusedSide{x, e, nullptr, nullptr, out_x, wq, wq + 2048, nullptr, nullptr, p->xe_b, p->gx_as, p->gx_an, p->gx_b, p->ne_n_val, (int)N, (int)E, rem_x};
     a.side[1] = uds::FusedSide{e, x, nullptr, nullptr, out_e, wq + 8192, wq + 10240, nullptr, nullptr, p->ex_b, p->ge_as, p->ge_an, p->ge_b, p->ne_e_val, (int)E, (int)N, rem_e};
     a.S = (int)S;
@@ -1673,6 +1753,7 @@
     const uint4 *w_small_n = wq, *w_big_n = wq + 768, *w_small_e = wq + 768 + 2048, *w_big_e = wq + 2 * 768 + 2048;
     uds::FusedArgs a;
     a.blocks = nullptr;
+    a.xteam = nullptr;
     const bool has32 = fx == 64 && fe == 64;
     a.side[0] = uds::FusedSide{x, e, xb, eb, out_x, w_small_n, w_big_n, has32 ? wq + WS_BIG32_OFF : nullptr, has32 ? wq + WS_SMALL32_OFF : nullptr, p->xe_b, p->gx_as, p->gx_an, p->gx_b, p->ne_n_val, (int)N, (int)E, rem_x};
     a.side[1] = uds::FusedSide{e, x, eb, xb, out_e, w_small_e, w_big_e, has32 ? wq + WS_BIG32_OFF + WS_BIG32_LEN : nullptr, has32 ? wq + WS_SMALL32_OFF + WS_SMALL32_LEN : nullptr, p->ex_b, p->ge_as, p->ge_an, p->ge_b, p->ne_e_val, (int)E, (int)N, rem_e};
@@ -1685,6 +1766,7 @@
       a.q_cap = u.plan.q_cap;
       a.meta_cap = u.blk_cap;
       a.blocks = side < 0 ? u.d_blocks : u.d_blocks_side[side];
+      a.xteam = side < 0 ? u.d_xteam : nullptr;
       lds_need = u.lds_bytes;
     };
     use_plan(sl, -1);
@@ -1695,7 +1777,7 @@
     a.dbg = reinterpret_cast<unsigned long long *>(ws + PACKED_WEIGHT_FLOATS);
 #endif
     auto set_chunk = [&](int64_t working_tiles) {
-      int64_t chunk = pick_chunk(S, working_tiles);
+      int64_t chunk = (flags & UDS_FLAG_ONE_CHUNK) ? S : pick_chunk(S, working_tiles);
 #ifdef UDS_KNOBS
       if (const char *ov = std::getenv("UDS_CHUNK")) chunk = std::max<int64_t>(1, std::min<int64_t>(S, std::atoll(ov)));
 #endif
@@ -1706,7 +1788,7 @@
       a.side_mask = 3;
       const int grid = set_chunk(a.n_tiles);
       const int64_t ws_lds = uds::fused_ws_lds_bytes(a.p_cap, a.q_cap, a.meta_cap);
-      bool ws = fx == 64 && !xb && !eb && ws_lds <= FUSED_LDS_BUDGET && a.p_cap <= 128 && a.q_cap <= 256;
+      bool ws = fx == 64 && !xb && !eb && ws_lds <= FUSED_LDS_BUDGET && a.p_cap <= 128 && a.q_cap <= 256 && a.xteam;
 #ifdef UDS_KNOBS
       if (std::getenv("UDS_NO_WS")) ws = false;
 #endif
diff --git a/include/uds_hip.h b/include/uds_hip.h
--- a/include/uds_hip.h
+++ b/include/uds_hip.h
@@ -287,6 +287,10 @@
 int uds_tile_plan_sizes(const uds_tile_plan_t *plan, int64_t *n_tiles, int64_t *pool_len, int32_t *caps3);
 int uds_tile_plan_copy(const uds_tile_plan_t *plan, int32_t *hdr_out, int32_t *pool_out);
 int uds_tile_plan_blocks(const uds_tile_plan_t *plan, int32_t *blocks_out, int64_t *stride_out);
+int uds_tile_plan_xteam(const uds_tile_plan_t *plan, int32_t *out );
+int uds_tile_plan_xteam_load(const uds_tile_plan_t *plan, const int32_t *table, int32_t *load_out );
+int uds_network_set_xteam(uds_network_t *net, const int32_t *table);
+int uds_network_get_xteam(const uds_network_t *net, int32_t *units_out , int32_t *table_out );
 
 typedef struct uds_spatial_params {
   const float *xe_k, *xe_b;
@@ -304,7 +308,8 @@
 
 enum {
   UDS_FLAG_EXACT_FP32 = 1,
-  UDS_FLAG_REQUIRE_FUSED = 2
+  UDS_FLAG_REQUIRE_FUSED = 2,
+  UDS_FLAG_ONE_CHUNK = 4
 };
 
 int64_t uds_spatial_workspace_floats(const uds_network_t *net, int64_t S, int64_t h, int64_t d);
```

Result: no change. 294,800 (median of 6 runs) (+0.7%).
